# theislab/dca

Measured on AMD Instinct MI355X. Metric: cells/sec training (ZINB AE, 68k x 20k), higher is better.
Workload: dtype f32

## Files before the change

dca_amd/build.py:

```python
import os
import shutil
import subprocess
import sys

HERE = os.path.dirname(os.path.abspath(__file__))
ROOT = os.path.dirname(HERE)
CSRC = os.path.join(HERE, 'csrc')
LIB = os.path.join(CSRC, 'libdcahip.so')
SOURCES = ['dcahip_zinb.hip', 'dcahip_gemm.hip', 'dcahip_layers.hip', 'dcahip_heads.hip', 'dcahip_prep.hip', 'dcahip_opt.hip',
           'dcahip_dropout.hip', 'dcahip_sparse.hip', 'dcahip_peer.hip', 'dcahip_knn.hip', 'dcahip_kmeans.hip', 'dcahip_gram.hip',
           'dcahip_silhouette.hip']
HEADERS = ['zinb_math.hpp', 'h2_math.hpp', 'philox.hpp', 'knn_dist.hpp']
ARCH = 'gfx950'
HOST_LIB = os.path.join(CSRC, 'libdcahost.so')
HOST_SOURCES = ['dcahost_tsv.cpp', 'dcahost_read.cpp']


def _hipcc():
    for c in (shutil.which('hipcc'), '/opt/rocm/bin/hipcc'):
        if c and os.path.exists(c):
            return c
    raise RuntimeError('hipcc not found: cannot build libdcahip.so')


def _deps():
    return [os.path.join(CSRC, s) for s in SOURCES + HEADERS] + [os.path.join(ROOT, 'include', 'dcahip.h')]


def source_fingerprint():
    import hashlib
    h = hashlib.sha256()
    for d in _deps():
        h.update(os.path.basename(d).encode())
        if os.path.exists(d):
            with open(d, 'rb') as f:
                h.update(f.read())
    return h.hexdigest()


def needs_build():
    if not os.path.exists(LIB):
        return True
    t = os.path.getmtime(LIB)
    if any(os.path.exists(d) and os.path.getmtime(d) > t for d in _deps()):
        return True
    try:
        with open(LIB + '.src') as f:
            return f.read().strip() != source_fingerprint()
    except OSError:
        return True


def _obj_path(src, tag):
    return os.path.join(CSRC, '_obj', os.path.basename(src) + ('.' + tag if tag else '') + '.o')


def _obj_fingerprint(src, hdrs, defines):
    import hashlib
    h = hashlib.sha256()
    for d in [src] + list(hdrs):
        h.update(os.path.basename(d).encode())
        with open(d, 'rb') as f:
            h.update(f.read())
    h.update('\0'.join(defines).encode())
    return h.hexdigest()
# ... 74 lines not shown
```

dca_amd/config.py:

```python
import os
from dataclasses import dataclass, fields


def _flag(name, default):
    v = os.environ.get(name)
    return default if v is None else v not in ('0', '', 'off', 'false', 'False')


@dataclass
class EngineConfig:
    stack: str = 'steps'
    bwd_chain: bool = True
    wide_planes: bool = True
    wide_h2: bool = True
    dp_sharded_opt: bool = False
    dp_graph: bool = True
    dp_peer_exchange: bool = False
    device_prep: bool = True
    fused_write: bool = True
    resident: str = 'auto'
    counts_compact: bool = False
    graph_steps: int = 8
    sparse_dw_min: int = 512
    lut_fwd_min: int = 1024
    enc0_nt_min: int = 256
    predict_chunk: int = 1024

    _ENV = {'stack': 'DCA_AMD_STACK', 'bwd_chain': 'DCA_AMD_BWD_CHAIN', 'wide_planes': 'DCA_AMD_WIDE_PLANES', 'wide_h2': 'DCA_AMD_WIDE_H2',
            'dp_sharded_opt': 'DCA_AMD_DP_SHARDED_OPT', 'dp_graph': 'DCA_AMD_DP_GRAPH', 'device_prep': 'DCA_AMD_DEVICE_PREP',
            'fused_write': 'DCA_AMD_FUSED_WRITE', 'dp_peer_exchange': 'DCA_AMD_DP_PEER', 'resident': 'DCA_AMD_RESIDENT',
            'counts_compact': 'DCA_AMD_COUNTS_COMPACT'}

    @classmethod
    def from_env(cls):
        c = cls()
        for f in fields(cls):
            env = cls._ENV.get(f.name)
            if env is None:
                continue
            if f.type is bool or isinstance(getattr(c, f.name), bool):
                setattr(c, f.name, _flag(env, getattr(c, f.name)))
            elif os.environ.get(env) is not None:
                setattr(c, f.name, type(getattr(c, f.name))(os.environ[env]))
        if c.stack not in ('steps', 'coop', 'off'):
            raise ValueError('DCA_AMD_STACK must be steps, coop or off (got %r)' % c.stack)
        if c.resident not in ('auto', 'counts', 'dense'):
            raise ValueError('DCA_AMD_RESIDENT must be auto, counts or dense (got %r)' % c.resident)
        return c


def current():
    return EngineConfig.from_env()
```

dca_amd/csrc/dcahip_heads.hip:

```cpp
#include <hip/hip_runtime.h>
#include <stdint.h>
#include <type_traits>
#include "dcahip.h"
#include "zinb_math.hpp"

namespace {

using f32x16 = __attribute__((ext_vector_type(16))) float;

constexpr int kTG = 32;
constexpr int kTR = 32;
constexpr int kLdS = 33;
constexpr int kWG = 2;
constexpr int kMaxGrid = 2048;
constexpr int kMaxSmallGrid = 8192;
constexpr int kCUs = 256;
constexpr int kZU = 4;
constexpr int kQCap = 320;

__device__ __forceinline__ int rowmap(int e, int hi) { return (e & 3) + 8 * (e >> 2) + 4 * hi; }

__device__ __forceinline__ void wave_sync() {
    __builtin_amdgcn_fence(__ATOMIC_RELEASE, "wavefront");
    __builtin_amdgcn_wave_barrier();
    __builtin_amdgcn_fence(__ATOMIC_ACQUIRE, "wavefront");
}

using f16x8 = __attribute__((ext_vector_type(8))) _Float16;
using f16x2v = __attribute__((ext_vector_type(2))) _Float16;
using f32x2v = __attribute__((ext_vector_type(2))) float;
using u32x4 = __attribute__((ext_vector_type(4))) unsigned;
using u32x2 = __attribute__((ext_vector_type(2))) unsigned;
using s16x4 = __attribute__((ext_vector_type(4))) short;

constexpr int kWR2 = 8;
constexpr int kWr8MinNT = 5;
constexpr int kHTile = 2 * 32 * 64;
constexpr int kTop = 13;
constexpr int kDExp0 = 8;
constexpr float kDLim = 30000.f;
constexpr int kDSlack = 2;
constexpr int kEHZero = 64;

#define MFMAH(a, b, c) __builtin_amdgcn_mfma_f32_32x32x16_f16(__builtin_bit_cast(f16x8, a), __builtin_bit_cast(f16x8, b), c, 0, 0, 0)

__device__ __forceinline__ unsigned pk_f16(float a, float b) {
    return __builtin_bit_cast(unsigned, __builtin_convertvector(f32x2v{a, b}, f16x2v));
}
__device__ __forceinline__ float resid_lo(unsigned p, float x) {
    float r;
    asm("v_fma_mix_f32 %0, %1, -1.0, %2 op_sel:[0,0,0] op_sel_hi:[1,0,0]" : "=v"(r) : "v"(p), "v"(x));
    return r;
}
__device__ __forceinline__ float resid_hi(unsigned p, float x) {
    float r;
    asm("v_fma_mix_f32 %0, %1, -1.0, %2 op_sel:[1,0,0] op_sel_hi:[1,0,0]" : "=v"(r) : "v"(p), "v"(x));
    return r;
// ... 711 lines not shown
#pragma unroll
                for (int h = 0; h < NH; ++h) bsum[h] += rs[(n++) * 64];
                thsum += rs[(n++) * 64];
            }
            __syncthreads();
        }
    }
    if (r == 0 && tile_ok) {
        const bool direct = p.S == 1;
        float* out = direct ? p.gW : p.ws_dw + (long)s * p.dw_stride;
        const long ldo = direct ? p.ldg : p.ldws;
        const float fin = direct ? p.inv_n : 1.f;
        const bool cw = gene < p.plane;
#pragma unroll
        for (int h = 0; h < NH; ++h) {
#pragma unroll
            for (int ib = 0; ib < 2; ++ib)
#pragma unroll
                for (int e = 0; e < 16; ++e) {
                    const int i = ib * 32 + rowmap(e, hi);
                    if (cw && i < p.hL) out[(long)i * ldo + (long)h * p.plane + gene] = dW[h][ib][e] * fin;
                }
            const float bv = bsum[h] + __shfl_xor(bsum[h], 32, 64);
            if (cw && hi == 0) out[(long)p.hL * ldo + (long)h * p.plane + gene] = bv * fin;
        }
        if (CONST_DISP) {
            const float tv = thsum + __shfl_xor(thsum, 32, 64);
            if (direct) {
                if (gvalid && hi == 0) {
                    const float e = expf(p.theta_w[gene]);
                    p.g_theta[gene] = (e >= 1e-3f && e <= 1e4f) ? tv * p.inv_n * e : 0.f;
                }
            } else if (cw && hi == 0) {
                out[(long)(p.hL + 1) * ldo + gene] = tv;
            }
        }
    }
    __syncthreads();
    first_item = false;
    }

#pragma unroll
    for (int off = 32; off > 0; off >>= 1) dacc += __shfl_down(dacc, off, 64);
    if (lane == 0) lred[wave] = dacc;
    __syncthreads();
    if (tid == 0) {
        double v = 0.0;
        for (int w = 0; w < WR; ++w) v += lred[w];
        p.partials[blockIdx.x] = v;
    }
}


struct ReduceDwArgs {
    const float* ws; int S; long stride; int hL; long ldws, ncols; float* gW; long ldg;
    const float* theta_w; float* g_theta; int G;
    float scale;
    const float* ws2; int S2; const int* tail_tiles; int ntail; long plane;
    int tail_first;
};

__device__ __forceinline__ void reduce_dw_body(const ReduceDwArgs& q, int bid, int nblk) {
    const int hL = q.hL;
    const long ldws = q.ldws, ncols = q.ncols; float* gW = q.gW; const long ldg = q.ldg;
    const float* theta_w = q.theta_w; float* g_theta = q.g_theta; const int G = q.G;
    const float sc = q.scale;
    __shared__ unsigned tailbm[kMaxGrid / 32];
    if (q.ntail > 0) {
        for (int i = threadIdx.x; i < kMaxGrid / 32; i += 256) tailbm[i] = 0u;
        __syncthreads();
        for (int i = threadIdx.x; i < q.ntail; i += 256) {
            const int tl = q.tail_tiles ? q.tail_tiles[i] : q.tail_first + i;
            if (tl >= 0 && tl < kMaxGrid) atomicOr(&tailbm[tl >> 5], 1u << (tl & 31));
        }
        __syncthreads();
    }
    auto is_tail = [&](long col_in_plane) { const int tl = (int)(col_in_plane / kTG); return q.ntail > 0 && ((tailbm[tl >> 5] >> (tl & 31)) & 1u); };
    if ((ncols & 3) == 0 && (ldws & 3) == 0 && (ldg & 3) == 0 && (q.stride & 3) == 0 && (q.plane & 3) == 0 &&
        ((reinterpret_cast<uintptr_t>(q.ws) | reinterpret_cast<uintptr_t>(gW) | reinterpret_cast<uintptr_t>(q.ws2)) & 15) == 0) {
        const long nq = ncols >> 2, totalq = (long)(hL + 1) * nq;
        for (long idx = (long)bid * 256 + threadIdx.x; idx < totalq; idx += (long)nblk * 256) {
            const long i = idx / nq, c = (idx - i * nq) << 2;
            const bool tl = is_tail(c % q.plane);
            const float* ws = tl ? q.ws2 : q.ws; const int S = tl ? q.S2 : q.S; const long stride = q.stride;
            float4 v = *reinterpret_cast<const float4*>(ws + i * ldws + c);
            for (int s = 1; s < S; ++s) {
                const float4 x = *reinterpret_cast<const float4*>(ws + (long)s * stride + i * ldws + c);
                v.x += x.x; v.y += x.y; v.z += x.z; v.w += x.w;
            }
            v.x *= sc; v.y *= sc; v.z *= sc; v.w *= sc;
            *reinterpret_cast<float4*>(gW + i * ldg + c) = v;
        }
    } else {
        const long total = (long)(hL + 1) * ncols;
        for (long idx = (long)bid * 256 + threadIdx.x; idx < total; idx += (long)nblk * 256) {
            const long i = idx / ncols, c = idx - i * ncols;
            const bool tl = is_tail(c % q.plane);
            const float* ws = tl ? q.ws2 : q.ws; const int S = tl ? q.S2 : q.S;
            float v = 0.f;
            for (int s = 0; s < S; ++s) v += ws[(long)s * q.stride + i * ldws + c];
            gW[i * ldg + c] = v * sc;
        }
    }
    if (g_theta) {
        for (long c = (long)bid * 256 + threadIdx.x; c < G; c += (long)nblk * 256) {
            const bool tl = is_tail(c);
            const float* ws = tl ? q.ws2 : q.ws; const int S = tl ? q.S2 : q.S; const long stride = q.stride;
            float v = 0.f;
            for (int s = 0; s < S; ++s) v += ws[(long)s * stride + (long)(hL + 1) * ldws + c];
            const float e = expf(theta_w[c]);
            g_theta[c] = (e >= 1e-3f && e <= 1e4f) ? v * sc * e : 0.f;
        }
    }
}

__global__ __launch_bounds__(256) void heads_reduce_dw_kernel(ReduceDwArgs q) { reduce_dw_body(q, blockIdx.x, gridDim.x); }

struct ReduceDhArgs {
    const float* ws; int ntg, B, Bpad, KT, hL; float* dH; long lddh; float scale;
    const double* loss_partials; int n_partials; double loss_scale; float* loss_out;
    const float* ws2; int ntg2;
};

template <int GL>
__device__ __forceinline__ void reduce_dh_body(const ReduceDhArgs& q, int bid) {
    const float* ws = q.ws; const int ntg = q.ntg, B = q.B, KT = q.KT, hL = q.hL; float* dH = q.dH; const long lddh = q.lddh;
    const double* loss_partials = q.loss_partials; const int n_partials = q.n_partials; const double loss_scale = q.loss_scale;
    float* loss_out = q.loss_out;
    constexpr int OUT = 256 / GL;
    __shared__ float4 red[256];
    const int o = threadIdx.x % OUT, gl = threadIdx.x / OUT;
    const int q4 = KT / 4;
    const long nq = (long)B * q4;
    const long quad = (long)bid * OUT + o;
    float4 v = make_float4(0.f, 0.f, 0.f, 0.f);
    if (quad < nq) {
        const long tq = (long)kTR * q4;
        const long t = quad / tq, within = quad - t * tq;
        const float4* src = reinterpret_cast<const float4*>(ws) + t * ntg * tq + within;
        for (int gt0 = gl; gt0 < ntg; gt0 += 8 * GL) {
            float4 x[8];
#pragma unroll
            for (int u = 0; u < 8; ++u) {
                const int gt = gt0 + u * GL;
                x[u] = src[(long)(gt < ntg ? gt : gl) * tq];
            }
#pragma unroll
            for (int u = 0; u < 8; ++u)
                if (gt0 + u * GL < ntg) { v.x += x[u].x; v.y += x[u].y; v.z += x[u].z; v.w += x[u].w; }
        }
        if (q.ntg2 > 0) {
            const float4* src2 = reinterpret_cast<const float4*>(q.ws2) + t * q.ntg2 * tq + within;
            for (int gt = gl; gt < q.ntg2; gt += GL) { const float4 x = src2[(long)gt * tq]; v.x += x.x; v.y += x.y; v.z += x.z; v.w += x.w; }
        }
    }
    red[threadIdx.x] = v;
    __syncthreads();
    if (gl == 0 && quad < nq) {
#pragma unroll
        for (int k = 1; k < GL; ++k) {
            const float4 x = red[k * OUT + o];
            v.x += x.x; v.y += x.y; v.z += x.z; v.w += x.w;
        }
        const long row = quad / q4;
        const int i = (int)(quad - row * q4) * 4;
        float* d = dH + row * lddh + i;
        if (i + 0 < hL) d[0] = v.x * q.scale;
        if (i + 1 < hL) d[1] = v.y * q.scale;
        if (i + 2 < hL) d[2] = v.z * q.scale;
        if (i + 3 < hL) d[3] = v.w * q.scale;
    }
    if (loss_out && bid == 0) {
        __shared__ double lsum[256];
        double a = 0.0;
        for (int i = threadIdx.x; i < n_partials; i += 256) a += loss_partials[i];
        lsum[threadIdx.x] = a;
        __syncthreads();
        for (int st = 128; st > 0; st >>= 1) {
            if ((int)threadIdx.x < st) lsum[threadIdx.x] += lsum[threadIdx.x + st];
            __syncthreads();
        }
        if (threadIdx.x == 0) {
            float lf = (float)(lsum[0] * loss_scale);
            if (isnan(lf)) lf = INFINITY;
            *loss_out = lf;
        }
    }
}

template <int GL>
__global__ __launch_bounds__(256) void heads_reduce_dh_kernel(ReduceDhArgs q) { reduce_dh_body<GL>(q, blockIdx.x); }

template <int GL>
__global__ __launch_bounds__(256) void heads_reduce_both_kernel(ReduceDhArgs qh, ReduceDwArgs qw, int n_dh) {
    if ((int)blockIdx.x < n_dh) reduce_dh_body<GL>(qh, blockIdx.x);
    else reduce_dw_body(qw, blockIdx.x - n_dh, gridDim.x - n_dh);
}


struct HeadsPlan {
    bool small;
    int HLB, WR, S, NT, ntg, ngb, grid;
    int nitems, npart;
    long ldws, dw_stride, dw_bytes, dh_bytes, hs_bytes;
    int nmain, ntail, S2, grid2, npart2, nitems2;
    long dh2_bytes, dw2_bytes;
};

inline bool al16(const void* p) { return (reinterpret_cast<uintptr_t>(p) & 15) == 0; }

bool make_heads_plan(int B, int hL, int G, long plane, int flags, HeadsPlan* out) {
    if (flags & (DCAHIP_NLL_POISSON | DCAHIP_NLL_MSE)) return false;
    if (B <= 0 || G <= 0 || hL <= 0 || hL > 64 || plane < G || (plane & 3) || plane > ((G + 31) & ~31)) return false;
    if (B > (1 << 22)) return false;
    const bool has_pi = flags & DCAHIP_NLL_HAS_PI, cdisp = flags & DCAHIP_NLL_CONST_DISP;
    const int NH = 1 + (cdisp ? 0 : 1) + (has_pi ? 1 : 0);
    HeadsPlan p;
    p.HLB = 2;
    p.NT = (B + kTR - 1) / kTR;
    p.ntg = (G + kTG - 1) / kTG;
    p.ngb = p.ntg;
    if (p.ngb > kMaxGrid) return false;
    p.small = p.NT < kWr8MinNT;
    static_assert((kWr8MinNT - 1) * kMaxGrid <= kMaxSmallGrid, "loss partials of the four-wave kernel");
    p.WR = p.small ? 1 : kWR2;
    const int smax = (p.NT + p.WR - 1) / p.WR;
    double best = 1e300;
    p.S = 1;
    const double item_cost = 0.75;
    for (int S = 1; S <= smax && (long)S * p.ngb <= kMaxGrid; ++S) {
        const long items = (long)S * p.ngb;
        const long rounds = (items + kCUs - 1) / kCUs;
        const int tiles = (p.NT + S * p.WR - 1) / (S * p.WR);
        const double cost = (double)rounds * (tiles + item_cost);
        if (cost < best - 1e-9) { best = cost; p.S = S; }
    }
    p.nitems = p.S * p.ngb;
    p.grid = p.nitems;
    p.npart = p.ntg;
    if (p.small) {
        p.S = p.NT;
        p.nitems = p.NT * p.ntg;
        p.grid = p.nitems;
        p.npart = p.ntg;
    } else {
        const int res = kCUs / p.S * p.S;
        if (p.grid > res) p.grid = res;
        p.npart = p.grid / p.S;
    }
// ... 441 lines not shown
        }
    const int ea = block_exp(wave_max(ma)), eb = block_exp(wave_max(mb));
    const float sa = pow2i(ea), sb = pow2i(eb);
    f32x16 acc;
#pragma unroll
    for (int e = 0; e < 16; ++e) acc[e] = 0.f;
    for (int k0 = 0; k0 < K; k0 += 16) {
        float av[8], bv[8];
#pragma unroll
        for (int j = 0; j < 8; ++j) {
            av[j] = A[(long)l31 * K + k0 + 8 * hi + j] * sa;
            bv[j] = B[(long)(k0 + 8 * hi + j) * 32 + l31] * sb;
        }
        u32x4 af[2], bf[2];
        split8(av, af);
        split8(bv, bf);
        MFMA_H3(af, bf, acc)
    }
    const float un = pow2i(-(ea + eb));
#pragma unroll
    for (int e = 0; e < 16; ++e) C[rowmap(e, hi) * 32 + l31] = acc[e] * un;
}

template <bool P, bool C, bool YC>
void launch_fused(const HeadsPlan& pl, const HeadsArgs2& a, hipStream_t s) {
    if (pl.small) hipLaunchKernelGGL((heads_fused_small_kernel<P, C, YC>), dim3(pl.grid), dim3(256), 0, s, a);
    else hipLaunchKernelGGL((heads_fused_h2_kernel<P, C, YC>), dim3(pl.grid), dim3(64 * kWR2), 0, s, a);
}

}

extern "C" long dcahip_heads_fused_workspace_bytes(int B, int hL, int G, long plane, int flags) {
    HeadsPlan p;
    if (!make_heads_plan(B, hL, G, plane, flags, &p)) return 0;
    long need = 0;
    for (int nt = 1; nt <= p.NT; ++nt) {
        const int b = nt * kTR < B ? nt * kTR : B;
        HeadsPlan q;
        if (!make_heads_plan(b, hL, G, plane, flags, &q)) continue;
        const long n = q.dw_bytes + q.dh_bytes + q.hs_bytes + q.dw2_bytes + q.dh2_bytes;
        if (n > need) need = n;
    }
    return need;
}

extern "C" int dcahip_x3_product_32x32(const float* A, const float* B, float* C, int K, void* stream) {
    if (!A || !B || !C || K <= 0 || (K & 15)) return DCAHIP_EINVAL;
    hipLaunchKernelGGL(x3_product_kernel, dim3(1), dim3(64), 0, static_cast<hipStream_t>(stream), A, B, C, K);
    return (int)hipGetLastError();
}

extern "C" int dcahip_heads_tile_order_len(int G) { return G > 0 ? (((G + kTG - 1) / kTG + kWG - 1) / kWG) * kWG : 0; }

extern "C" int dcahip_heads_fused(const float* H, long ldh, const float* Wh, long ldw,
                                  const float* bh, long plane, const float* theta_w,
                                  const float* y, long ldy,
                                  const unsigned char* yc, long ldc, const int* ovf_ptr, const int* ovf_col,
                                  const float* ovf_val, const float* sf, const int* perm,
                                  const long long* cursor, int B, int hL, int G, float ridge,
                                  float inv_n, int flags, float* gW, long ldg, float* g_theta,
                                  float* dH, long lddh, double* loss_partials, int* n_partials_out,
                                  void* workspace, long workspace_bytes, const int* tile_order,
                                  float* loss_out, int d_exp, void* stream) {
    const bool has_pi = flags & DCAHIP_NLL_HAS_PI, cdisp = flags & DCAHIP_NLL_CONST_DISP;
    HeadsPlan pl;
    if (!make_heads_plan(B, hL, G, plane, flags, &pl)) return DCAHIP_EINVAL;
    if (!H || !Wh || !bh || (!y && !yc) || !sf || !gW || !dH || !loss_partials || !workspace) return DCAHIP_EINVAL;
    if (cdisp && (!theta_w || !g_theta)) return DCAHIP_EINVAL;
    if (workspace_bytes < pl.dw_bytes + pl.dh_bytes + pl.hs_bytes + pl.dw2_bytes + pl.dh2_bytes) return DCAHIP_EINVAL;
    if (!al16(H) || !al16(Wh) || !al16(workspace) || (ldh & 3) || (ldw & 3) || ldh < ((hL + 3) & ~3))
        return DCAHIP_EINVAL;
    if (d_exp > 0 || d_exp < -24 || !(ridge >= 0.f) || ridge > 1e3f) return DCAHIP_EINVAL;
    const int NH = 1 + (cdisp ? 0 : 1) + (has_pi ? 1 : 0);
    if (ldw < (long)NH * plane || ldg < (long)NH * plane) return DCAHIP_EINVAL;
    if (yc ? (ldc < G || ldc > 0xffffffffL) : (ldy < G || ldy > 0xffffffffL)) return DCAHIP_EINVAL;
    float* ws_dh = static_cast<float*>(workspace);
    float* ws_dw = ws_dh + pl.dh_bytes / sizeof(float);
    float* ws_dh2 = ws_dw + pl.dw_bytes / sizeof(float);
    float* ws_dw2 = ws_dh2 + pl.dh2_bytes / sizeof(float);
    hipStream_t s = static_cast<hipStream_t>(stream);
    bool direct_dw = false;
    {
        unsigned short* HA = reinterpret_cast<unsigned short*>(reinterpret_cast<char*>(workspace) + pl.dh_bytes + pl.dw_bytes +
                                                               pl.dh2_bytes + pl.dw2_bytes);
        unsigned short* HT = HA + (long)pl.NT * kHTile;
        int* eH = reinterpret_cast<int*>(HT + (long)pl.NT * kHTile);
        if (!pl.small) {
            hipLaunchKernelGGL(heads_split_h_kernel, dim3(pl.NT), dim3(256), 0, s, H, ldh, B, hL, HA, HT, eH);
            int rc0 = (int)hipGetLastError();
            if (rc0 != 0) return rc0;
        }
        direct_dw = pl.S == 1;
        HeadsArgs2 a{HA, HT, eH, H, ldh, gW, ldg, g_theta, Wh, ldw, bh, theta_w, y, ldy, yc, ldc, ovf_ptr, ovf_col, ovf_val,
                     sf, perm, cursor, ws_dw, pl.dw_stride, ws_dh,
                     pl.npart, pl.nitems, tile_order, loss_partials, plane, pl.ldws, B, hL, G, pl.S, pl.NT, ridge, inv_n, d_exp, 0};
        auto launch = [&](const HeadsPlan& q, const HeadsArgs2& b) {
            if (yc) {
                if (has_pi && cdisp) launch_fused<true, true, true>(q, b, s);
                else if (has_pi) launch_fused<true, false, true>(q, b, s);
                else if (cdisp) launch_fused<false, true, true>(q, b, s);
                else launch_fused<false, false, true>(q, b, s);
            } else {
                if (has_pi && cdisp) launch_fused<true, true, false>(q, b, s);
                else if (has_pi) launch_fused<true, false, false>(q, b, s);
                else if (cdisp) launch_fused<false, true, false>(q, b, s);
                else launch_fused<false, false, false>(q, b, s);
            }
        };
        launch(pl, a);
        if (pl.ntail > 0) {
            HeadsPlan q2 = pl;
            q2.grid = pl.grid2; q2.S = pl.S2;
            HeadsArgs2 b = a;
            b.ws_dw = ws_dw2; b.ws_dh = ws_dh2; b.npart = pl.npart2; b.nitems = pl.nitems2; b.S = pl.S2;
            b.partials = loss_partials + pl.grid; b.tile_base = pl.nmain;
            launch(q2, b);
        }
    }
    int rc = (int)hipGetLastError();
    if (rc != 0) return rc;
    const int n_part = pl.grid + pl.grid2;
    if (n_partials_out) *n_partials_out = n_part;
    {
        const int KT = pl.HLB * 32;
        const long nq = (long)B * (KT / 4);
        const ReduceDhArgs qh{ws_dh, pl.npart, B, pl.NT * kTR, KT, hL, dH, lddh, inv_n, loss_partials, n_part, (double)inv_n, loss_out,
                              ws_dh2, pl.npart2};
        const long total = (long)(hL + 1) * pl.ldws;
        long gr = (total / 4 + 255) / 256;
        if (gr > 2048) gr = 2048;
        if (gr < 1) gr = 1;
        const ReduceDwArgs qw{ws_dw, pl.S, pl.dw_stride, hL, pl.ldws, pl.ldws, gW, ldg, cdisp ? theta_w : nullptr,
                              cdisp ? g_theta : nullptr, G, inv_n,
                              ws_dw2, pl.S2, (pl.ntail > 0 && tile_order) ? tile_order + pl.nmain : nullptr, pl.ntail, plane, pl.nmain};
        const int gl = (nq <= 1024 && pl.npart >= 256) ? 64 : (nq >= 64L * 512 ? 4 : 16);
        const int n_dh = (int)((nq + 256 / gl - 1) / (256 / gl));
        if (!direct_dw) {
            const dim3 grid(n_dh + (int)gr);
            if (gl == 64) hipLaunchKernelGGL(heads_reduce_both_kernel<64>, grid, dim3(256), 0, s, qh, qw, n_dh);
            else if (gl == 4) hipLaunchKernelGGL(heads_reduce_both_kernel<4>, grid, dim3(256), 0, s, qh, qw, n_dh);
            else hipLaunchKernelGGL(heads_reduce_both_kernel<16>, grid, dim3(256), 0, s, qh, qw, n_dh);
        } else {
            if (gl == 64) hipLaunchKernelGGL(heads_reduce_dh_kernel<64>, dim3(n_dh), dim3(256), 0, s, qh);
            else if (gl == 4) hipLaunchKernelGGL(heads_reduce_dh_kernel<4>, dim3(n_dh), dim3(256), 0, s, qh);
            else hipLaunchKernelGGL(heads_reduce_dh_kernel<16>, dim3(n_dh), dim3(256), 0, s, qh);
        }
        rc = (int)hipGetLastError();
    }
    return rc;
}
```

dca_amd/csrc/dcahip_layers.hip:

```cpp
#include <hip/hip_runtime.h>
#include <stdint.h>
#include "dcahip.h"

namespace {

constexpr int kMaxChunks = 256;
constexpr int kApplyRows = 16;

constexpr float kSeluScale = 1.0507009873554805f, kSeluAlpha = 1.6732632423543772f;
constexpr int kActPre = 12;

__device__ __attribute__((noinline)) float act_fwd_other(int a, float x) {
    switch (a) {
        case 2: return tanhf(x);
        case 3: { const float e = expf(-fabsf(x)); const float s = 1.f / (1.f + e); return x >= 0.f ? s : e * s; }
        case 4: return x > 0.f ? x : expm1f(x);
        case 5: return kSeluScale * (x > 0.f ? x : kSeluAlpha * expm1f(x));
        case 6: return fmaxf(x, 0.f) + log1pf(expf(-fabsf(x)));
        case 7: return x / (1.f + fabsf(x));
        case 10: return fminf(fmaxf(0.2f * x + 0.5f, 0.f), 1.f);
        case 11: return expf(x);
        case 12: { const float e = expf(-fabsf(x)); const float s = 1.f / (1.f + e); return x * (x >= 0.f ? s : e * s); }
        case 13: return 0.5f * x * (1.f + erff(x * 0.70710678118654752f));
        default: return x > 0.f ? x : 0.3f * x;
    }
}
__device__ __forceinline__ float act_fwd(int a, float x) {
    if (a == 1) return fmaxf(x, 0.f);
    if (a == 0) return x;
    return act_fwd_other(a, x);
}

__device__ __attribute__((noinline)) float act_grad_other(int a, float v) {
    switch (a) {
        case 2: return 1.f - v * v;
        case 3: return v * (1.f - v);
        case 4: return v > 0.f ? 1.f : v + 1.f;
        case 5: return v > 0.f ? kSeluScale : v + kSeluScale * kSeluAlpha;
        case 6: return -expm1f(-v);
        case 7: { const float t = 1.f - fabsf(v); return t * t; }
        case 10: return v > 0.f && v < 1.f ? 0.2f : 0.f;
        case 11: return v;
        case 12: {
            const float e = expf(-fabsf(v)); const float s0 = 1.f / (1.f + e); const float s = v >= 0.f ? s0 : e * s0;
            return s * (1.f + v * (1.f - s));
        }
        case 13:
            return 0.5f * (1.f + erff(v * 0.70710678118654752f)) + v * 0.39894228040143268f * expf(-0.5f * v * v);
        default: return v > 0.f ? 1.f : 0.3f;
    }
}
__device__ __forceinline__ float act_grad(int a, float h) {
    if (a == 1) return h > 0.f ? 1.f : 0.f;
    if (a == 0) return 1.f;
    return act_grad_other(a, h);
// ... 795 lines not shown
                    const int r = wg + kBwdWGs * (ty + 4 * j);
                    acc[j] = fmaf(r < a.B ? dZs[r][c] : 0.f, w, acc[j]);
                }
            }
#pragma unroll
            for (int j = 0; j < NR; ++j) {
                const int r = wg + kBwdWGs * (ty + 4 * j);
                if (r < a.B) a.dHp[(long)r * a.lddp + k] = acc[j];
            }
        }
    }
}

__global__ __launch_bounds__(256) void relu_bwd_kernel(const float* dH, long ldd, const float* Hact,
                                                       long ldh, int B, int H, float* dZ, long ldz, int act) {
    const long total = (long)B * H;
    for (long i = (long)blockIdx.x * 256 + threadIdx.x; i < total; i += (long)gridDim.x * 256) {
        const int r = (int)(i / H), c = (int)(i - (long)r * H);
        dZ[(long)r * ldz + c] = dH[(long)r * ldd + c] * act_grad(act, Hact[(long)r * ldh + c]);
    }
}

__global__ __launch_bounds__(256) void relu_fwd_kernel(const float* Z, long ldz, int B, int H,
                                                       float* Hout, long ldh, int act) {
    const long total = (long)B * H;
    for (long i = (long)blockIdx.x * 256 + threadIdx.x; i < total; i += (long)gridDim.x * 256) {
        const int r = (int)(i / H), c = (int)(i - (long)r * H);
        Hout[(long)r * ldh + c] = act_fwd(act, Z[(long)r * ldz + c]);
    }
}

__global__ __launch_bounds__(256) void colsum_chain_kernel(const float* x, long ldx, int B, int N,
                                                           const float* theta_w, float* out) {
    __shared__ float sm[256];
    const int tx = threadIdx.x & 63, ty = threadIdx.x >> 6;
    const int c = blockIdx.x * 64 + tx;
    float s = 0.f;
    if (c < N) for (int i = ty; i < B; i += 4) s += x[(long)i * ldx + c];
    const float tot = wg_rowlane_sum(s, sm);
    if (c < N && ty == 0) {
        float chain = 1.f;
        if (theta_w) {
            const float e = expf(theta_w[c]);
            chain = (e >= 1e-3f && e <= 1e4f) ? e : 0.f;
        }
        out[c] = tot * chain;
    }
}

struct StepEnd {
    const float* loss; double weight; float* hist; int rows_per_slot; double* acc; long long* cursor; int advance; int on;
};

__global__ __launch_bounds__(256) void rmsprop_clip_kernel(float* w, const float* g, float* ms,
                                                           long n, const float* lrp, float rho,
                                                           float eps, float clip, StepEnd se) {
    if (se.on && blockIdx.x == 0 && threadIdx.x == 0) {
        const long long c = se.cursor ? *se.cursor : 0;
        if (se.loss) {
            const float l = *se.loss;
            if (se.hist) se.hist[se.rows_per_slot > 0 ? c / se.rows_per_slot : 0] = l;
            if (se.acc) *se.acc += (double)l * se.weight;
        }
        if (se.cursor) *se.cursor = c + se.advance;
    }
    const float lr = *lrp;
    const long nv = n >> 2;
    const long stride = (long)gridDim.x * 256;
    for (long i = (long)blockIdx.x * 256 + threadIdx.x; i < nv; i += stride) {
        float4 gv = reinterpret_cast<const float4*>(g)[i];
        float4 mv = reinterpret_cast<const float4*>(ms)[i];
        float4 wv = reinterpret_cast<const float4*>(w)[i];
        float* gp = &gv.x; float* mp = &mv.x; float* wp = &wv.x;
#pragma unroll
        for (int j = 0; j < 4; ++j) {
            float gj = gp[j];
            if (clip > 0.f) gj = fminf(fmaxf(gj, -clip), clip);
            mp[j] = rho * mp[j] + (1.f - rho) * gj * gj;
            wp[j] = wp[j] - lr * gj / (sqrtf(mp[j]) + eps);
        }
        reinterpret_cast<float4*>(ms)[i] = mv;
        reinterpret_cast<float4*>(w)[i] = wv;
    }
    for (long i = (nv << 2) + (long)blockIdx.x * 256 + threadIdx.x; i < n; i += stride) {
        float gj = g[i];
        if (clip > 0.f) gj = fminf(fmaxf(gj, -clip), clip);
        const float m = rho * ms[i] + (1.f - rho) * gj * gj;
        ms[i] = m;
        w[i] = w[i] - lr * gj / (sqrtf(m) + eps);
    }
}

__global__ __launch_bounds__(256) void transpose_kernel(const float* __restrict__ src, long lds_, int R, int C,
                                                        float* __restrict__ dst, long ldd,
                                                        const int* __restrict__ perm, const long long* __restrict__ cursor) {
    __shared__ float tile[32][33];
    const int tx = threadIdx.x & 31, ty = threadIdx.x >> 5;
    const int r0 = blockIdx.y * 32, c0 = blockIdx.x * 32;
    const long long cur = (perm && cursor) ? *cursor : 0;
#pragma unroll
    for (int k = 0; k < 4; ++k) {
        const int r = r0 + ty + 8 * k, c = c0 + tx;
        float v = 0.f;
        if (r < R && c < C) {
            const long sr = perm ? (long)perm[cur + r] : (long)r;
            v = src[sr * lds_ + c];
        }
        tile[ty + 8 * k][tx] = v;
    }
    __syncthreads();
#pragma unroll
    for (int k = 0; k < 4; ++k) {
        const int c = c0 + ty + 8 * k, r = r0 + tx;
        if (c < C && r < R) dst[(long)c * ldd + r] = tile[tx][ty + 8 * k];
    }
}

__global__ __launch_bounds__(256) void transpose64_kernel(const float* __restrict__ src, long lds_, int R, int C,
                                                          float* __restrict__ dst, long ldd,
                                                          const int* __restrict__ perm, const long long* __restrict__ cursor) {
    __shared__ float tile[64][65];
    const int tq = threadIdx.x & 15, tr = threadIdx.x >> 4;
    const int r0 = blockIdx.y * 64, c0 = blockIdx.x * 64;
    const long long cur = (perm && cursor) ? *cursor : 0;
    float4 v[4];
#pragma unroll
    for (int k = 0; k < 4; ++k) {
        const int r = r0 + tr + 16 * k, c = c0 + 4 * tq;
        const int rc = r < R ? r : R - 1;
        const long sr = perm ? (long)perm[cur + rc] : (long)rc;
        v[k] = *reinterpret_cast<const float4*>(src + sr * lds_ + (c < C ? c : 0));
    }
#pragma unroll
    for (int k = 0; k < 4; ++k) {
        const int r = tr + 16 * k, c = 4 * tq;
        tile[r][c] = v[k].x; tile[r][c + 1] = v[k].y; tile[r][c + 2] = v[k].z; tile[r][c + 3] = v[k].w;
    }
    __syncthreads();
#pragma unroll
    for (int k = 0; k < 4; ++k) {
        const int c = tr + 16 * k, r = 4 * tq;
        if (c0 + c < C) {
// ... 176 lines not shown
                if (L.xhat) L.xhat[(long)(r0 + r) * L.ldx + c] = xh;
                L.Hout[(long)(r0 + r) * L.ldh + c] = h;
                ht[r * kStackLd + c] = h;
            }
        }
        if (i + 1 == a.n) break;
        const SmallLayer& N = a.l[i + 1];
        const int K = H, HN = N.H;
        for (int idx = tid; idx < ((K + 3) & ~3) * 64; idx += 256) {
            const int k = idx >> 6, cc = idx & 63;
            wl[k * kStackLd + cc] = (k < K && cc < HN) ? N.W[(long)k * N.ldw + cc] : 0.f;
        }
        for (int idx = tid; idx < kStackRows * 4; idx += 256) {
            const int r = idx >> 2, kk = (K & ~3) + (idx & 3);
            if (kk >= K && kk < ((K + 3) & ~3)) ht[r * kStackLd + kk] = 0.f;
        }
        __syncthreads();
        float acc[kStackRows / 4];
#pragma unroll
        for (int j = 0; j < kStackRows / 4; ++j) acc[j] = 0.f;
        const int K4 = (K + 3) & ~3;
        for (int k = 0; k < K4; k += 4) {
            const float w0 = wl[(k + 0) * kStackLd + c], w1 = wl[(k + 1) * kStackLd + c];
            const float w2 = wl[(k + 2) * kStackLd + c], w3 = wl[(k + 3) * kStackLd + c];
#pragma unroll
            for (int j = 0; j < kStackRows / 4; ++j) {
                const int r = ty + 4 * j;
                if (r < nrows) {
                    const float4 h4 = *reinterpret_cast<const float4*>(ht + r * kStackLd + k);
                    acc[j] = fmaf(h4.w, w3, fmaf(h4.z, w2, fmaf(h4.y, w1, fmaf(h4.x, w0, acc[j]))));
                }
            }
        }
        __syncthreads();
        if (c < HN) {
            const float b = N.bias ? N.bias[c] : 0.f;
#pragma unroll
            for (int j = 0; j < kStackRows / 4; ++j) {
                const int r = ty + 4 * j;
                if (r < nrows) {
                    const float z = acc[j] + b;
                    zt[r * kStackLd + c] = z;
                    if (N.Z) N.Z[(long)(r0 + r) * N.ldz + c] = z;
                }
            }
        }
        __syncthreads();
        block_stats(i + 1);
        fresh = true;
    }
    if (nbar) grid_exit(a.sync, (unsigned)nwg);
}

__global__ __launch_bounds__(256) void hidden_stack_bwd_kernel(StackBwdArgs a) {
    __shared__ __attribute__((aligned(16))) float dyt[kStackRows * kStackLd];
    __shared__ __attribute__((aligned(16))) float xt[kStackRows * kStackLd];
    __shared__ __attribute__((aligned(16))) float ht[kStackRows * kStackLd];
    __shared__ __attribute__((aligned(16))) float wl[64 * kStackLd];
    __shared__ float smf[256];
    const int tid = threadIdx.x, tx = tid & 63, ty = tid >> 6;
    const int wg = blockIdx.x, nwg = a.nwg;
    const int cr = chunk_rows(a.B, nwg);
    const int r0 = wg * cr;
    const int nrows = max(0, min(a.B, r0 + cr) - r0);
    const int c = tx;
    unsigned nbar = 0;
    auto prep = [&](int i, bool load_dh, bool with_sums) {
        const StackBwdLayer& L = a.l[i];
        const int H = L.H;
        if (load_dh) {
            for (int r = ty; r < kStackRows; r += 4)
                dyt[r * kStackLd + tx] = (r < nrows && tx < H) ? L.dHin[(long)(r0 + r) * L.lddh + tx] : 0.f;
        }
        float s1 = 0.f, s2 = 0.f;
        const float bc = c < H ? pre_beta(a.act, L.beta, c) : 0.f;
        if (c < H)
            for (int r = ty; r < nrows; r += 4) {
                const float h = L.Hact[(long)(r0 + r) * L.ldh + c];
                const float xh = L.xhat[(long)(r0 + r) * L.ldx + c];
                const float dy = dyt[r * kStackLd + c] * act_slope(a.act, h, xh, bc);
                dyt[r * kStackLd + c] = dy;
                xt[r * kStackLd + c] = xh;
                s1 += dy; s2 += dy * xh;
            }
        if (!with_sums) { __syncthreads(); return; }
        const float t1 = wg_rowlane_sum(s1, smf);
        const float t2 = wg_rowlane_sum(s2, smf);
        float* part = a.part + (long)i * nwg * 2 * 64;
        if (c < H && ty == 0) {
            part[((long)wg * 2 + 0) * H + c] = t1;
            part[((long)wg * 2 + 1) * H + c] = t2;
        }
    };
    bool fresh = false, have_tile = false;
    if (a.first == 0) { prep(a.n - 1, true, true); fresh = true; have_tile = true; }
    for (int step = max(a.first, 1); step <= min(a.last, a.n); ++step) {
        const int i = a.n - step;
        const StackBwdLayer& L = a.l[i];
        const int H = L.H;
        if (!have_tile) { prep(i, true, false); have_tile = true; }
        if (fresh) grid_barrier(a.sync, (unsigned)nwg * (++nbar));
        const float* part = a.part + (long)i * nwg * 2 * 64;
        float v1 = 0.f, v2 = 0.f;
        {
            const int cc = c < H ? c : H - 1;
            for (int e0 = ty; e0 < nwg; e0 += 64) {
// ... 34 lines not shown
        {
            float acc[16];
#pragma unroll
            for (int j = 0; j < 16; ++j) acc[j] = 0.f;
            float bs = 0.f;
            for (int r = 0; r < nrows; ++r) {
                const float d = dyt[r * kStackLd + c];
                bs += d;
#pragma unroll
                for (int q4 = 0; q4 < 4; ++q4) {
                    const float4 h4 = *reinterpret_cast<const float4*>(ht + r * kStackLd + 16 * ty + 4 * q4);
                    acc[4 * q4 + 0] = fmaf(h4.x, d, acc[4 * q4 + 0]); acc[4 * q4 + 1] = fmaf(h4.y, d, acc[4 * q4 + 1]);
                    acc[4 * q4 + 2] = fmaf(h4.z, d, acc[4 * q4 + 2]); acc[4 * q4 + 3] = fmaf(h4.w, d, acc[4 * q4 + 3]);
                }
            }
#pragma unroll
            for (int j = 0; j < 16; ++j) {
                const int k = 16 * ty + j;
                if (k < K) gw[(long)k * 64 + c] = acc[j];
            }
            if (ty == 0) gw[(long)K * 64 + c] = bs;
        }
        {
            float acc[kStackRows / 4];
#pragma unroll
            for (int j = 0; j < kStackRows / 4; ++j) acc[j] = 0.f;
            for (int c4 = 0; c4 < 64; c4 += 4) {
                const float4 w4 = *reinterpret_cast<const float4*>(wl + tx * kStackLd + c4);
#pragma unroll
                for (int j = 0; j < kStackRows / 4; ++j) {
                    const int r = ty + 4 * j;
                    if (r < nrows) {
                        const float4 d4 = *reinterpret_cast<const float4*>(dyt + r * kStackLd + c4);
                        acc[j] = fmaf(d4.w, w4.w, fmaf(d4.z, w4.z, fmaf(d4.y, w4.y, fmaf(d4.x, w4.x, acc[j]))));
                    }
                }
            }
            __syncthreads();
            const StackBwdLayer& P = a.l[i - 1];
#pragma unroll
            for (int j = 0; j < kStackRows / 4; ++j) {
                const int r = ty + 4 * j;
                const float v = (r < nrows && tx < K) ? acc[j] : 0.f;
                dyt[r * kStackLd + tx] = v;
                if (r < nrows && tx < K && P.dHin) P.dHin[(long)(r0 + r) * P.lddh + tx] = v;
            }
        }
        __syncthreads();
        prep(i - 1, false, true);
        fresh = true;
    }
    if (a.last > a.n) {
        if (fresh) grid_barrier(a.sync, (unsigned)nwg * (++nbar));
        for (int i = 1; i < a.n; ++i) {
            const StackBwdLayer& L = a.l[i];
            const int total = (L.K + 1) * L.H;
            const float* gw = a.gwp + (long)i * nwg * 65 * 64;
            const int el = tid & 31, sl = tid >> 5;
            const int per = (nwg + 7) / 8;
            for (int e0 = wg * 32; e0 < total; e0 += nwg * 32) {
                const int e = e0 + el;
                const int ec = e < total ? e : total - 1;
                const int k = ec / L.H, cc = ec - k * L.H;
                const float* src = gw + (long)k * 64 + cc;
                float v = 0.f;
                for (int b0 = sl * per; b0 < min(nwg, (sl + 1) * per); b0 += 16) {
                    float pv[16];
#pragma unroll
                    for (int u = 0; u < 16; ++u) pv[u] = src[(long)min(b0 + u, nwg - 1) * 65 * 64];
#pragma unroll
                    for (int u = 0; u < 16; ++u) if (b0 + u < min(nwg, (sl + 1) * per)) v += pv[u];
                }
                __syncthreads();
                smf[tid] = v;
                __syncthreads();
                if (tid < 32 && e < total) {
                    float t = 0.f;
#pragma unroll
                    for (int q8 = 0; q8 < 8; ++q8) t += smf[q8 * 32 + tid];
                    L.gW[(long)k * L.ldg + cc] = t;
                }
            }
        }
    }
    if (nbar) grid_exit(a.sync, (unsigned)nwg);
}

__device__ __forceinline__ bool w_tile_vec(const float* W, long ldw, int H) {
    return (H & 3) == 0 && (ldw & 3) == 0 && (reinterpret_cast<uintptr_t>(W) & 15) == 0;
}
template <int VEC = 0>
__device__ __forceinline__ void w_tile_request(const float* W, long ldw, int K, int H, int tid, float4 (&wv)[4]) {
    if (VEC == 0 && (!W || K <= 0)) {
#pragma unroll
        for (int q = 0; q < 4; ++q) wv[q] = make_float4(0.f, 0.f, 0.f, 0.f);
        return;
    }
    const bool vec = VEC == 1 || (VEC == 0 && w_tile_vec(W, ldw, H));
    if (vec) {
#pragma unroll
        for (int q = 0; q < 4; ++q) {
            const int idx = tid + 256 * q, k = min(idx >> 4, K - 1), c4 = min((idx & 15) * 4, H - 4);
            wv[q] = *reinterpret_cast<const float4*>(W + (long)k * ldw + c4);
        }
    } else {
#pragma unroll
        for (int q = 0; q < 4; ++q) {
            const int idx = tid + 256 * q, k = min(idx >> 4, K - 1), c4 = (idx & 15) * 4;
            const float* src = W + (long)k * ldw;
            wv[q].x = src[min(c4 + 0, H - 1)]; wv[q].y = src[min(c4 + 1, H - 1)];
            wv[q].z = src[min(c4 + 2, H - 1)]; wv[q].w = src[min(c4 + 3, H - 1)];
        }
    }
}
__device__ __forceinline__ void w_tile_store(float* wl, int K, int H, int tid, const float4 (&wv)[4]) {
#pragma unroll
    for (int q = 0; q < 4; ++q) {
        const int idx = tid + 256 * q, k = idx >> 4, c4 = (idx & 15) * 4;
        float4 v = wv[q];
        if (k >= K || c4 + 0 >= H) v.x = 0.f;
        if (k >= K || c4 + 1 >= H) v.y = 0.f;
        if (k >= K || c4 + 2 >= H) v.z = 0.f;
        if (k >= K || c4 + 3 >= H) v.w = 0.f;
        *reinterpret_cast<float4*>(wl + k * kStackLd + c4) = v;
    }
}

constexpr int kStepRows = 32;

struct StepFwdArgs {
    SmallLayer cur, nxt;
    int B, act, nwg, stats_only;
    float momentum, eps;
    const float* part_in;
    float* part_out;
    const float* ext_in; const float* ext_counts; int ext_E;
};

// ... 75 lines not shown
            float h = 0.f;
            if (r < nrows && c < H) {
                const float xh = bn_xhat(z[j], mean, inv);
                h = act_fwd(a.act, xh + beta);
                if (L.xhat) L.xhat[(long)(r0 + r) * L.ldx + c] = xh;
                L.Hout[(long)(r0 + r) * L.ldh + c] = h;
            }
            ht[r * kStackLd + c] = h;
        }
        if (!N.W) return;
        w_tile_store(wl, K, HN, tid, wv);
        __syncthreads();
        float acc[kStepRows / 4];
#pragma unroll
        for (int j = 0; j < kStepRows / 4; ++j) acc[j] = 0.f;
        tile_fwd<kStepRows / 4, kStackLd, kStackLd, 0>(acc, wl, ht, (K + 3) & ~3, tx, ty);
        Hs = HN;
#pragma unroll
        for (int j = 0; j < kStepRows / 4; ++j) {
            const int r = ty + 4 * j;
            out_z[j] = acc[j] + nbias;
            if (r < nrows && c < HN && N.Z) N.Z[(long)(r0 + r) * N.ldz + c] = out_z[j];
        }
    } else {
#pragma unroll
        for (int j = 0; j < kStepRows / 4; ++j) out_z[j] = z[j];
    }
    float sv = 0.f;
#pragma unroll
    for (int j = 0; j < kStepRows / 4; ++j) if (ty + 4 * j < nrows && c < Hs) sv += out_z[j];
    const float tot = wg_rowlane_sum(sv, smf);
    const float bmean = nrows > 0 ? tot / (float)nrows : 0.f;
    float q = 0.f;
#pragma unroll
    for (int j = 0; j < kStepRows / 4; ++j) if (ty + 4 * j < nrows && c < Hs) { const float d = out_z[j] - bmean; q += d * d; }
    const float bm2 = wg_rowlane_sum(q, smf);
    if (c < Hs && ty == 0) {
        a.part_out[((long)wg * 2 + 0) * Hs + c] = bmean;
        a.part_out[((long)wg * 2 + 1) * Hs + c] = bm2;
    }
}

struct StepBwdArgs {
    StackBwdLayer cur, low;
    int B, act, nwg, sums_only;
    float n_total;
    float* dZ0; long ldz0;
    const float* part_in;
    float* part_out;
    float* gwp;
    const float* ext_in;
};

__global__ __launch_bounds__(256) void stack_bwd_step_kernel(StepBwdArgs a) {
    __shared__ __attribute__((aligned(16))) float dyt[kStepRows * kStackLd];
    __shared__ __attribute__((aligned(16))) float ht[kStepRows * kStackLd];
    __shared__ __attribute__((aligned(16))) float wl[64 * kStackLd];
    __shared__ float smf[256];
    const int tid = threadIdx.x, tx = tid & 63, ty = tid >> 6;
    const int wg = blockIdx.x, E = a.nwg;
    const int cr = chunk_rows(a.B, E);
    const int r0 = wg * cr;
    const int nrows = max(0, min(a.B, r0 + cr) - r0);
    const int c = tx;
    const StackBwdLayer& L = a.cur;
    const int H = L.H, cc = c < H ? c : H - 1;
    float dh[kStepRows / 4], hv[kStepRows / 4], xv[kStepRows / 4];
#pragma unroll
    for (int j = 0; j < kStepRows / 4; ++j) {
        const int r = ty + 4 * j;
        const long row = r0 + (r < nrows ? r : (nrows > 0 ? nrows - 1 : 0));
        dh[j] = L.dHin[row * L.lddh + cc]; hv[j] = L.Hact[row * L.ldh + cc]; xv[j] = L.xhat[row * L.ldx + cc];
    }
    float dy[kStepRows / 4];
    const float bc = pre_beta(a.act, L.beta, cc);
    if (a.sums_only) {
        float s1 = 0.f, s2 = 0.f;
        tile_dy_sums(dy, xv, c < H, nrows, ty, [&](int j) { return dh[j] * act_slope(a.act, hv[j], xv[j], bc); }, s1, s2);
        const float t1 = wg_rowlane_sum(s1, smf), t2 = wg_rowlane_sum(s2, smf);
        if (c < H && ty == 0) { a.part_out[((long)wg * 2 + 0) * H + c] = t1; a.part_out[((long)wg * 2 + 1) * H + c] = t2; }
        return;
    }
    const float* const ein = a.ext_in ? a.ext_in : a.part_in;
    const int Em = a.ext_in ? 1 : E;
    float p1[16], p2[16];
#pragma unroll
    for (int u = 0; u < 16; ++u) {
        const long eo = (long)(ty + 4 * u < Em ? ty + 4 * u : Em - 1) * 2;
        p1[u] = ein[(eo + 0) * H + cc]; p2[u] = ein[(eo + 1) * H + cc];
    }
    const bool has_low = a.low.Hact != nullptr;
    const int K = has_low ? L.K : 0;
    float4 wv[4];
    float hp[kStepRows / 4];
    w_tile_request(has_low ? L.W : nullptr, L.ldw, K, H, tid, wv);
#pragma unroll
    for (int j = 0; j < kStepRows / 4; ++j) {
        const int r = ty + 4 * j;
        const long row = r0 + (r < nrows ? r : (nrows > 0 ? nrows - 1 : 0));
        const int kc = tx < K ? tx : (K > 0 ? K - 1 : 0);
        hp[j] = has_low ? L.Hprev[row * L.ldp + kc] : 0.f;
    }
    const float inv = L.inv_std[cc];
    float v1 = 0.f, v2 = 0.f;
#pragma unroll
    for (int u = 0; u < 16; ++u) if (ty + 4 * u < Em && c < H) { v1 += p1[u]; v2 += p2[u]; }
#pragma unroll 1
    for (int e0 = ty + 64; e0 < Em; e0 += 64) {
        float q1[16], q2[16];
#pragma unroll
        for (int u = 0; u < 16; ++u) {
            const long eo = (long)(e0 + 4 * u < Em ? e0 + 4 * u : Em - 1) * 2;
            q1[u] = ein[(eo + 0) * H + cc]; q2[u] = ein[(eo + 1) * H + cc];
// ... 10 lines not shown
        const int r = ty + 4 * j;
        float dz = 0.f;
        if (r < nrows && c < H) {
            dz = bn_dz(inv, dh[j] * act_slope(a.act, hv[j], xv[j], bc), xv[j], m1, m2);
            if (!has_low) a.dZ0[(long)(r0 + r) * a.ldz0 + c] = dz;
        }
        dyt[r * kStackLd + c] = dz;
        ht[r * kStackLd + tx] = (r < nrows && tx < K) ? hp[j] : 0.f;
    }
    if (!has_low) return;
    w_tile_store(wl, K, H, tid, wv);
    __syncthreads();
    float lh[kStepRows / 4], lx[kStepRows / 4];
#pragma unroll
    for (int j = 0; j < kStepRows / 4; ++j) {
        const int r = ty + 4 * j;
        const long row = r0 + (r < nrows ? r : (nrows > 0 ? nrows - 1 : 0));
        const int kc = tx < K ? tx : (K > 0 ? K - 1 : 0);
        lh[j] = a.low.Hact[row * a.low.ldh + kc];
        lx[j] = a.low.xhat[row * a.low.ldx + kc];
    }
    float* gw = a.gwp + (long)wg * 65 * 64;
    {
        float acc[16];
#pragma unroll
        for (int j = 0; j < 16; ++j) acc[j] = 0.f;
        float bs = 0.f;
        tile_dw<kStackLd, 2>(acc, bs, dyt, ht, nrows, tx, ty);
#pragma unroll
        for (int j = 0; j < 16; ++j) {
            const int k = 16 * ty + j;
            if (k < K) gw[(long)k * 64 + c] = acc[j];
        }
        if (ty == 0) gw[(long)K * 64 + c] = bs;
    }
    float acc[kStepRows / 4];
#pragma unroll
    for (int j = 0; j < kStepRows / 4; ++j) acc[j] = 0.f;
    tile_dhp<kStepRows / 4, kStackLd, 2>(acc, wl, dyt, tx, ty);
    const StackBwdLayer& P = a.low;
    const float pbc = pre_beta(a.act, P.beta, tx < K ? tx : (K > 0 ? K - 1 : 0));
    float s1 = 0.f, s2 = 0.f;
#pragma unroll
    for (int j = 0; j < kStepRows / 4; ++j) {
        const int r = ty + 4 * j;
        if (r < nrows && tx < K) {
            P.dHin[(long)(r0 + r) * P.lddh + tx] = acc[j];
            const float d = acc[j] * act_slope(a.act, lh[j], lx[j], pbc);
            s1 += d; s2 += d * lx[j];
        }
    }
    const float t1 = wg_rowlane_sum(s1, smf), t2 = wg_rowlane_sum(s2, smf);
    if (tx < K && ty == 0) { a.part_out[((long)wg * 2 + 0) * K + tx] = t1; a.part_out[((long)wg * 2 + 1) * K + tx] = t2; }
}

struct ChainBwdArgs {
    StackBwdLayer l[4];
    int B, act;
    float n_total;
    float* dZ0; long ldz0;
};

template <int NL, int R, bool VEC>
__global__ __launch_bounds__(256) void stack_bwd_chain_kernel(ChainBwdArgs a) {
    __shared__ __attribute__((aligned(16))) float dyt[4 * R * kStackLd];
    __shared__ __attribute__((aligned(16))) float ht[4 * R * kStackLd];
    __shared__ __attribute__((aligned(16))) float wl[64 * kStackLd];
    __shared__ float smf[256];
    const int tid = threadIdx.x, tx = tid & 63, ty = tid >> 6;
    const int nrows = a.B, c = tx;
    float hv[NL][R], xv[NL][R], inv[NL], dh[R];
    float4 wv[NL][4];
    {
        const StackBwdLayer& T = a.l[NL - 1];
        const int cc = c < T.H ? c : T.H - 1;
#pragma unroll
        for (int j = 0; j < R; ++j) {
            const int r = ty + 4 * j;
            dh[j] = T.dHin[(long)(r < nrows ? r : nrows - 1) * T.lddh + cc];
        }
    }
#pragma unroll
    for (int t = 0; t < NL; ++t) {
        const int i = NL - 1 - t;
        const StackBwdLayer& L = a.l[i];
        const int cc = c < L.H ? c : L.H - 1;
#pragma unroll
        for (int j = 0; j < R; ++j) {
            const int r = ty + 4 * j;
            const long row = r < nrows ? r : nrows - 1;
            hv[i][j] = L.Hact[row * L.ldh + cc]; xv[i][j] = L.xhat[row * L.ldx + cc];
        }
        inv[i] = L.inv_std[cc];
        if (i > 0) w_tile_request<VEC ? 1 : 2>(L.W, L.ldw, L.K, L.H, tid, wv[i]);
    }
#pragma unroll
    for (int t = 0; t < NL; ++t) {
        const int i = NL - 1 - t;
        const StackBwdLayer& L = a.l[i];
        const int H = L.H, K = i > 0 ? L.K : 0;
        float dy[R], s1 = 0.f, s2 = 0.f;
        if (a.act == 1) {
#pragma unroll
            for (int j = 0; j < R; ++j) dy[j] = hv[i][j] > 0.f ? dh[j] : 0.f;
        } else {
            const float bc = pre_beta(a.act, L.beta, c < H ? c : H - 1);
// ... 375 lines not shown
    if (!a_mean || !k || !c || !a_pi || B <= 0 || G <= 0 || lda < G || ldp < G) return DCAHIP_EINVAL;
    const int gy = B < 64 ? B : 64;
    hipLaunchKernelGGL(elempi_fwd_kernel, dim3((G + 255) / 256, gy), dim3(256), 0, static_cast<hipStream_t>(stream),
                       a_mean, lda, k, c, B, G, a_pi, ldp);
    return (int)hipGetLastError();
}

extern "C" int dcahip_elempi_bwd(const float* m, long lda, float* d_mean, const float* d_pi, long ldd, const float* k,
                                 int B, int G, float* gk, float* gc, double* workspace, void* stream) {
    if (!m || !d_mean || !d_pi || !k || !gk || !gc || !workspace || B <= 0 || G <= 0 || lda < G || ldd < G)
        return DCAHIP_EINVAL;
    const int R = B < kElemPiSlices ? B : kElemPiSlices;
    hipStream_t s = static_cast<hipStream_t>(stream);
    hipLaunchKernelGGL(elempi_bwd_kernel, dim3((G + 255) / 256, R), dim3(256), 0, s, m, lda, d_mean, d_pi, ldd, k, B, G,
                       workspace);
    hipLaunchKernelGGL(elempi_finish_kernel, dim3((G + 255) / 256), dim3(256), 0, s, workspace, R, G, gk, gc);
    return (int)hipGetLastError();
}

extern "C" int dcahip_bcast_cols(const float* s, long lds, int B, int G, float* out, long ldo, void* stream) {
    if (!s || !out || B <= 0 || G <= 0 || ldo < G || lds < 1) return DCAHIP_EINVAL;
    int gx = (G + 255) / 256;
    if (gx > 64) gx = 64;
    hipLaunchKernelGGL(bcast_cols_kernel, dim3(gx, B), dim3(256), 0, static_cast<hipStream_t>(stream), s, lds, B, G, out, ldo);
    return (int)hipGetLastError();
}

extern "C" int dcahip_row_sums_strided(const float* x, long ldx, int B, int G, float* out, long ldo, void* stream) {
    if (!x || !out || B <= 0 || G <= 0 || ldx < G || ldo < 1) return DCAHIP_EINVAL;
    hipLaunchKernelGGL(row_sums_strided_kernel, dim3((B + 3) / 4), dim3(256), 0, static_cast<hipStream_t>(stream),
                       x, ldx, B, G, out, ldo);
    return (int)hipGetLastError();
}

extern "C" int dcahip_colsum_chain(const float* x, long ldx, int B, int N, const float* theta_w,
                                   float* out, void* stream) {
    if (!x || !out || B <= 0 || N <= 0) return DCAHIP_EINVAL;
    hipLaunchKernelGGL(colsum_chain_kernel, dim3((N + 63) / 64), dim3(256), 0,
                       static_cast<hipStream_t>(stream), x, ldx, B, N, theta_w, out);
    return (int)hipGetLastError();
}

extern "C" int dcahip_rmsprop_clip(float* w, const float* g, float* ms, long n, const float* lr,
                                   float rho, float eps, float clip, const float* loss, double weight,
                                   float* hist, int rows_per_slot, double* acc, long long* cursor, int advance,
                                   void* stream) {
    if (!w || !g || !ms || !lr || n <= 0) return DCAHIP_EINVAL;
    if (!al16(w) || !al16(g) || !al16(ms)) return DCAHIP_EINVAL;
    long grid = ((n >> 2) + 255) / 256;
    if (grid > 2048) grid = 2048;
    if (grid < 1) grid = 1;
    hipLaunchKernelGGL(rmsprop_clip_kernel, dim3((int)grid), dim3(256), 0,
                       static_cast<hipStream_t>(stream), w, g, ms, n, lr, rho, eps, clip,
                       StepEnd{loss, weight, hist, rows_per_slot, acc, cursor, advance, (loss || hist || acc || cursor) ? 1 : 0});
    return (int)hipGetLastError();
}

extern "C" int dcahip_hidden_stack_max_rows(void) { return kStackMaxWG * kStackRows; }

extern "C" long dcahip_hidden_stack_workspace_bytes(int n_layers, int B) {
    if (n_layers < 1 || n_layers > kStackMaxLayers || B <= 0 || B > kStackMaxWG * kStackRows) return 0;
    const long nwg = stack_workgroups(B, 16);
    return 256 + ((long)n_layers * nwg * 2 * 64 + (long)n_layers * nwg * 65 * 64) * (long)sizeof(float);
}

static int stack_plan(int n, int B, int rows_per_wg, int first, int last, int nsteps, int* nwg_out) {
    if (rows_per_wg < 16 || rows_per_wg > kStackRows || first < 0 || last < first || last >= nsteps) return DCAHIP_EINVAL;
    const int nwg = stack_workgroups(B, rows_per_wg);
    if (nwg > kStackMaxPhaseWG) return DCAHIP_EINVAL;
    if (last > first && nwg > kStackMaxWG) return DCAHIP_EINVAL;
    *nwg_out = nwg;
    return 0;
}

static bool stack_shape_ok(const void* layers, int n, int B) {
    return layers && n >= 1 && n <= kStackMaxLayers && B > 0 && B <= kStackMaxWG * kStackRows;
}

static bool stack_workspace_ok(const void* workspace, long workspace_bytes, int n, int B) {
    return workspace && workspace_bytes >= dcahip_hidden_stack_workspace_bytes(n, B) && al16(workspace);
}

static bool stack_fwd_layers(const dcahip_small_layer* layers, int n, bool need_z, SmallLayer* l) {
    for (int i = 0; i < n; ++i) {
        const dcahip_small_layer& q = layers[i];
        if (q.H <= 0 || q.H > 64 || !q.Hout || !q.moving_mean || !q.moving_var) return false;
        if (i == 0 ? !q.Z : (!q.W || q.K != layers[i - 1].H || (need_z && !q.Z))) return false;
        l[i] = small_layer(q);
    }
    return true;
}

static bool stack_bwd_layers(const dcahip_stack_bwd_layer* layers, int n, int act, bool need_dh, StackBwdLayer* l) {
    for (int i = 0; i < n; ++i) {
        const dcahip_stack_bwd_layer& q = layers[i];
        if (q.H <= 0 || q.H > 64 || !q.Hact || !q.xhat || !q.inv_std || (act >= kActPre && !q.beta)) return false;
        if (i > 0 && (!q.W || !q.Hprev || !q.gW || q.K != layers[i - 1].H || q.K > 64)) return false;
        if (!q.dH && (i == n - 1 || need_dh)) return false;
        l[i] = StackBwdLayer{q.W, q.ldw, q.K, q.H, q.Hact, q.ldh, q.xhat, q.ldx, q.inv_std, q.Hprev, q.ldp, q.gW, q.ldg,
                             q.dbeta, q.dH, q.lddh, q.beta};
    }
    return true;
}

static StepFwdArgs stack_fwd_step(const SmallLayer* l, int n, int B, float momentum, float eps, int act, int step, int nwg,
                                  float* part) {
// ... 72 lines not shown
                                            void* workspace, long workspace_bytes, void* stream) {
    if (!stack_shape_ok(layers, n, B) || !dZ0 || !stack_workspace_ok(workspace, workspace_bytes, n, B)) return DCAHIP_EINVAL;
    if (step < 0 || step > n || (step > 0 && !ext_sums)) return DCAHIP_EINVAL;
    const int nwg = stack_workgroups(B, kStepRows);
    if (nwg > kStackMaxPhaseWG) return DCAHIP_EINVAL;
    StackBwdLayer l[kStackMaxLayers];
    if (!stack_bwd_layers(layers, n, act, true, l)) return DCAHIP_EINVAL;
    float* part = reinterpret_cast<float*>(static_cast<char*>(workspace) + 256);
    StepBwdArgs q = stack_bwd_step(l, n, B, n_total, act, dZ0, ldz0, step, nwg, part);
    if (step > 0) q.ext_in = ext_sums;
    hipStream_t st = static_cast<hipStream_t>(stream);
    hipLaunchKernelGGL(stack_bwd_step_kernel, dim3(nwg), dim3(256), 0, st, q);
    const int made = stack_bwd_made(n, step);
    if (made >= 0 && sums_out)
        hipLaunchKernelGGL(stack_sums_combine_kernel, dim3(1), dim3(64), 0, st, (const float*)q.part_out, nwg, l[made].H, sums_out,
                           l[made].dbeta);
    return (int)hipGetLastError();
}

extern "C" int dcahip_hidden_stack_bwd(const dcahip_stack_bwd_layer* layers, int n, int B, float n_total, int act,
                                       float* dZ0, long ldz0, int rows_per_wg, int first_step, int last_step,
                                       void* workspace, long workspace_bytes, void* stream) {
    if (!stack_shape_ok(layers, n, B) || !dZ0) return DCAHIP_EINVAL;
    const bool one_launch = first_step == 0 && last_step == n + 1;
    const bool chain = one_launch && B <= kStackRows && n <= 4;
    if (!chain && !stack_workspace_ok(workspace, workspace_bytes, n, B)) return DCAHIP_EINVAL;
    StackBwdArgs a{};
    if (stack_plan(n, B, rows_per_wg, first_step, last_step, n + 2, &a.nwg)) return DCAHIP_EINVAL;
    if (!stack_bwd_layers(layers, n, act, !one_launch, a.l)) return DCAHIP_EINVAL;
    a.n = n; a.B = B; a.act = act; a.first = first_step; a.last = last_step; a.n_total = n_total;
    a.dZ0 = dZ0; a.ldz0 = ldz0;
    if (chain) {
        ChainBwdArgs q{};
        for (int i = 0; i < n; ++i) q.l[i] = a.l[i];
        q.B = B; q.act = act; q.n_total = n_total; q.dZ0 = dZ0; q.ldz0 = ldz0;
        bool vec = true;
        for (int i = 1; i < n; ++i) vec = vec && (q.l[i].H & 3) == 0 && (q.l[i].ldw & 3) == 0 && al16(q.l[i].W);
        hipStream_t st = static_cast<hipStream_t>(stream);
        if (B <= 32) { if (vec) launch_bwd_chain<8, true>(n, q, st); else launch_bwd_chain<8, false>(n, q, st); }
        else { if (vec) launch_bwd_chain<16, true>(n, q, st); else launch_bwd_chain<16, false>(n, q, st); }
        return (int)hipGetLastError();
    }
    a.sync = static_cast<unsigned*>(workspace);
    a.part = reinterpret_cast<float*>(static_cast<char*>(workspace) + 256);
    a.gwp = a.part + (long)n * a.nwg * 2 * 64;
    if (first_step == last_step && first_step <= n && rows_per_wg == kStepRows) {
        const StepBwdArgs q = stack_bwd_step(a.l, n, B, n_total, act, dZ0, ldz0, first_step, a.nwg, a.part);
        hipLaunchKernelGGL(stack_bwd_step_kernel, dim3(a.nwg), dim3(256), 0, static_cast<hipStream_t>(stream), q);
        return (int)hipGetLastError();
    }
    hipLaunchKernelGGL(hidden_stack_bwd_kernel, dim3(a.nwg), dim3(256), 0, static_cast<hipStream_t>(stream), a);
    return (int)hipGetLastError();
}
```

dca_amd/engine.py:

```python
import math

import numpy as np
import torch

from . import prep as _prep

BN_MOMENTUM = 0.99
BN_EPS = 1e-3
RMS_RHO = 0.9
RMS_EPS = 1e-7

AE_HEADS = {
    'zinb-conddisp': (('mean', 'disp', 'pi'), False),
    'zinb': (('mean', 'pi'), True),
    'nb-conddisp': (('mean', 'disp'), False),
    'nb': (('mean',), True),
    'poisson': (('mean',), False),
    'normal': (('mean',), False),
    'nb-shared': (('mean', 'disp'), False, ('disp',)),
    'zinb-shared': (('mean', 'disp', 'pi'), False, ('disp', 'pi')),
    'nb-fork': (('mean', 'disp'), False, ()),
    'zinb-fork': (('mean', 'disp', 'pi'), False, ()),
}
AE_FORK = ('nb-fork', 'zinb-fork')
# ... 90 lines not shown
    def all_reduce_sum_async(self, t):
        return None

    def wait(self, work):
        pass


def _truncated_normal(rng, stddev, shape):
    out = rng.normal(0.0, 1.0, size=shape)
    bad = np.abs(out) > 2.0
    while bad.any():
        out[bad] = rng.normal(0.0, 1.0, size=int(bad.sum()))
        bad = np.abs(out) > 2.0
    return out * stddev


KERAS_INITIALIZERS = ('glorot_uniform', 'glorot_normal', 'he_uniform', 'he_normal', 'lecun_uniform', 'lecun_normal',
                      'random_uniform', 'random_normal', 'truncated_normal', 'orthogonal', 'zeros', 'ones')


def keras_initializer(name, rng, fan_in, fan_out, shape=None):
    key = name.lower() if isinstance(name, str) else name
    vs = {'glorot_uniform': (1.0, 'avg', 'u'), 'glorot_normal': (1.0, 'avg', 'n'),
          'he_uniform': (2.0, 'in', 'u'), 'he_normal': (2.0, 'in', 'n'),
          'lecun_uniform': (1.0, 'in', 'u'), 'lecun_normal': (1.0, 'in', 'n')}
    shape = (fan_in, fan_out) if shape is None else shape
    if key in vs:
        scale, mode, distr = vs[key]
        n = (fan_in + fan_out) / 2.0 if mode == 'avg' else float(fan_in)
        if distr == 'u':
            lim = math.sqrt(3.0 * scale / n)
            w = rng.uniform(-lim, lim, size=shape)
        else:
            w = _truncated_normal(rng, math.sqrt(scale / n) / .87962566103423978, shape)
    elif key == 'random_uniform':
        w = rng.uniform(-0.05, 0.05, size=shape)
    elif key == 'random_normal':
        w = rng.normal(0.0, 0.05, size=shape)
    elif key == 'truncated_normal':
        w = _truncated_normal(rng, 0.05, shape)
    elif key == 'orthogonal' and len(shape) == 2:
        a = rng.normal(0.0, 1.0, size=(max(shape), min(shape)))
        q, r = np.linalg.qr(a)
        q = q * np.sign(np.diag(r))
        w = q if fan_in >= fan_out else q.T
    elif key == 'zeros':
        w = np.zeros(shape)
    elif key == 'ones':
        w = np.ones(shape)
    else:
        raise NotImplementedError('init=%r is not implemented on the MI355X path (available: %s)'
                                  % (name, ', '.join(KERAS_INITIALIZERS)))
    return np.ascontiguousarray(w, dtype=np.float32)


class ParamLayout:

    def __init__(self, ae_type, input_size, output_size, hidden_size, batchnorm, prelu=False):
        self.ae_type = ae_type
        self.prelu = bool(prelu)
        self.heads, self.const_disp = AE_HEADS[ae_type][:2]
        self.shared = AE_HEADS[ae_type][2] if len(AE_HEADS[ae_type]) > 2 else ()
        self.elempi = ae_type in AE_ELEMPI
        self.dense_heads = tuple(h for h in self.heads if not (self.elempi and h == 'pi'))
        self.planes = tuple(h for h in self.dense_heads if h not in self.shared)
        self.G_in, self.G_out = input_size, output_size
        self.Gp = _r4(output_size)
        self.NH = len(self.planes) * self.Gp + (4 if self.shared else 0)
        self.ldA = self.NH + (len(self.shared) + (1 if self.elempi else 0)) * self.Gp
        self.hidden = tuple(int(h) for h in hidden_size)
        self.center = int(np.floor(len(self.hidden) / 2.0))
        self.fork = len(self.heads) if ae_type in AE_FORK else 0
        self.hfork = 0
        if self.fork:
            if len(self.hidden) - 1 <= self.center:
                raise ValueError('%s needs at least one hidden layer behind the centre (the reference fails with '
                                 'AttributeError: last_hidden_mean)' % ae_type)
            self.hfork = self.hidden[-1]
            self.hidden = self.hidden[:self.center + 1] + (self.fork * self.hfork,)
        self.batchnorm = batchnorm
        self.seg = {}
        off = 0

        def add(name, shape, align=False):
            nonlocal off
            if align:
                off = _r4(off)
            self.seg[name] = (off, shape)
            off += int(np.prod(shape))

        fan_in = input_size
        for i, h in enumerate(self.hidden):
            add('W%d' % i, (fan_in, h), align=True)
            add('b%d' % i, (h,))
            if batchnorm:
                add('beta%d' % i, (h,))
            if self.prelu:
                add('alpha%d' % i, (h,))
            fan_in = h
        self.hL = self.hfork if self.fork else fan_in
        add('Wh', (self.hL, self.NH), align=True)
        add('bh', (self.NH,))
        if self.const_disp:
            add('theta_w', (self.Gp,), align=True)
        if self.elempi:
            add('pi_k', (self.Gp,), align=True)
# ... 65 lines not shown
        self.mv = [torch.ones(h, **f32) for h in lay.hidden] if batchnorm else []
        self.lr = torch.full((1,), 1e-3, **f32)
        self.cursor = torch.zeros(1, dtype=torch.int64, device=self.dev)
        self.acc = torch.zeros(2, dtype=torch.float64, device=self.dev)
        self.partials = torch.zeros(ops.max_partials, dtype=torch.float64, device=self.dev)
        self.val_loss_tmp = torch.zeros(1, **f32)
        self.clip = 5.0
        self.ldD = lay.ldA + (lay.Gp if lay.const_disp else 0)
        self.Bmax = 0
        self._hl = None
        self.X = self.Y = self.sf = self.perm = None
        self.has_targets = False
        self.csr = None
        self.out_cols = self.col_out = None
        self.perm_id = self.cursor0 = None
        self.tile_order = None
        self.hist = None
        self.prof = None
        self.use_fused = not (lay.shared or lay.fork or lay.elempi)
        self.sharedpi = bool(sharedpi) and lay.elempi
        self.ws_elempi = torch.zeros(ops.elempi_workspace_doubles(lay.G_out), dtype=torch.float64, device=self.dev) \
            if lay.elempi else None
        self.ws_heads = None
        self._pending = None
        self.W0T = None
        self.WhT = self.HT = self.XT = self.dZT = None
        self.pl = None
        self.opt_kind = 'rmsprop'
        self.slot2 = None
        self.m_sched = None
        self.opt_iter = torch.zeros(1, dtype=torch.int64, device=self.dev)
        self.reg = None
        self.reg_ws = None
        self._counts_world_key = None
        self._counts_local, self._counts_world = {}, {}
        n_conf = len(tuple(hidden_size))
        hd = list(hidden_dropout) if isinstance(hidden_dropout, (list, tuple)) else [hidden_dropout] * n_conf
        assert len(hd) == n_conf
        if lay.fork:
            hd = hd[:lay.center + 1] + [hd[-1]]
        self.drop = [float(r) for r in hd]
        self.in_drop = float(input_dropout)
        assert all(0.0 <= r < 1.0 for r in self.drop + [self.in_drop]), 'dropout rates must be in [0, 1)'
        self.has_dropout = any(r > 0.0 for r in self.drop) or self.in_drop > 0.0
        self.drop_seed = int(dropout_seed) & (2 ** 64 - 1)
        self.drop_iter = torch.zeros(1, dtype=torch.int64, device=self.dev)
        self.row0 = 0
        self.Xb = None
        self.cc = self.cc_in = None
        self.cc_csr = None
        self._tile_lut = False
        self.ws_enc0 = self.ws_enc0l = None
        self.ws_stack = None
        self.stack_mode = self.cfg.stack
        self.sparse_dw_min = self.cfg.sparse_dw_min

    def _t(self, name):
        return self.prof.section(name) if self.prof is not None else _NULL

    @property
    def _kperm(self):
        return self.perm_id if self.csr is not None else self.perm

    @property
    def _kcur(self):
        return self.cursor0 if self.csr is not None else self.cursor

    @property
    def _dhl(self):
        return self.dH[-1] if self.lay.hidden else self.dHin0

    def init_params(self, seed=0, init='glorot_uniform'):
        rng = np.random.RandomState(seed)
        lay = self.lay
        p = {}
        fan_in = lay.G_in
        for i, h in enumerate(lay.hidden):
            if lay.fork and i == len(lay.hidden) - 1:
                p['W%d' % i] = np.concatenate([keras_initializer(init, rng, fan_in, lay.hfork)
                                               for _ in range(lay.fork)], axis=1)
            else:
                p['W%d' % i] = keras_initializer(init, rng, fan_in, h)
            fan_in = h
        for hd in lay.dense_heads:
            p['W_' + hd] = keras_initializer(init, rng, lay.hL, 1 if hd in lay.shared else lay.G_out)
        if lay.elempi:
            units = 1 if self.sharedpi else lay.G_out
            k = keras_initializer(init, rng, units, units, shape=(units,))
            p['pi_k'] = np.full(lay.G_out, k[0], np.float32) if self.sharedpi else k
        self.set_params(p)

    def set_params(self, p):
        lay = self.lay
        w = self.w.cpu()
        for name, (off, shape) in lay.seg.items():
            if name in ('Wh', 'bh', 'theta_w', 'pi_k', 'pi_c'):
                continue
            if name in p:
                w[off:off + int(np.prod(shape))] = torch.as_tensor(
                    np.asarray(p[name], dtype=np.float32).reshape(-1))
        Wh = lay.view(w, 'Wh'); bh = lay.view(w, 'bh')
        for hd in lay.dense_heads:
            c0, c1 = lay.head_cols(hd)
            if 'W_' + hd in p:
                Wh[:, c0:c1] = torch.as_tensor(np.asarray(p['W_' + hd], dtype=np.float32))
            if 'b_' + hd in p:
# ... 887 lines not shown
            self.counts_world = cw
            self._counts_world_key = key
        self.row0 = int(sum(world_counts[:self.comm.rank]))

    def assert_finite(self, where=''):
        lay = self.lay
        bad = []
        if not bool(torch.isfinite(self.g[lay.P]).item()):
            bad.append('loss')
        if not bool(torch.isfinite(self.g[:lay.P]).all().item()) or not bool(torch.isfinite(self.w[:lay.P]).all().item()):
            for name in lay.seg:
                for flat, kind in ((self.g, 'gradient of '), (self.w, '')):
                    if not bool(torch.isfinite(lay.view(flat, name)).all().item()):
                        bad.append(kind + name)
        if bad:
            raise FloatingPointError('dca: %s has inf/nans%s' % (', '.join(bad), (' (' + where + ')') if where else ''))

    def train_step(self, B, B_global=None, world_counts=None, rows_per_slot=None):
        lay, ops, comm = self.lay, self.ops, self.comm
        Bg = B if B_global is None else B_global
        inv_n = 1.0 / (float(Bg) * lay.G_out)
        w, g = self.w, self.g
        if comm.dp:
            self.set_world_counts(world_counts)
        if B > 0:
            if self.csr is not None:
                with self._t('csr_gather'):
                    self._gather_step(B)
            self._forward_backward(B, Bg, inv_n)
        else:
            self._empty_step()
        if comm.dp and self._use_sharded_opt():
            sh = self.flat_len // comm.world
            lo = comm.rank * sh
            comm.all_reduce_sum(g[lay.P:lay.P + 1])
            gs = comm.reduce_scatter_sum(g, self._g_shard(sh))
            n_upd = max(0, min(sh, lay.P - lo))
            if n_upd > 0:
                with self._t('rmsprop_clip'):
                    ops.rmsprop_clip(w[lo:lo + sh], gs, self.ms[lo:lo + sh], n_upd, self.lr, RMS_RHO, RMS_EPS, self.clip)
            comm.all_gather_into(w, w[lo:lo + sh])
            if self.has_dropout:
                ops.counter_add(self.drop_iter, 1)
            ops.step_end(g[lay.P:], float(Bg), self.hist, rows_per_slot or max(self.Bmax, 1), self.acc, self.cursor, B)
            return
        if comm.dp:
            comm.all_reduce_sum(g[:lay.seg['Wh'][0]])
            if self._pending is not None:
                comm.wait(self._pending)
                self._pending = None
        if self.reg is not None:
            ops.l1l2_apply(self.reg, w, g, g[lay.P:], self.reg_ws)
        fused_end = self.opt_kind == 'rmsprop' and not self.has_dropout and hasattr(ops, 'rmsprop_clip_end')
        if fused_end:
            with self._t('rmsprop_clip'):
                ops.rmsprop_clip_end(w, g, self.ms, lay.P, self.lr, RMS_RHO, RMS_EPS, self.clip, g[lay.P:], float(Bg),
                                     self.hist, rows_per_slot or max(self.Bmax, 1), self.acc, self.cursor, B)
            return
        if self.opt_kind == 'rmsprop':
            with self._t('rmsprop_clip'):
                ops.rmsprop_clip(w, g, self.ms, lay.P, self.lr, RMS_RHO, RMS_EPS, self.clip)
        elif self.opt_kind == 'nadam':
            ops.nadam_step(w, g, self.ms, self.slot2, lay.P, self.lr, self.opt_iter, self.m_sched, self.clip)
            ops.counter_add(self.opt_iter, 1)
        else:
            ops.optimizer_step(self.opt_kind, w, g, None if self.opt_kind == 'sgd' else self.ms,
                               self.slot2, lay.P, self.lr, self.opt_iter, self.clip)
            ops.counter_add(self.opt_iter, 1)
        if self.has_dropout:
            ops.counter_add(self.drop_iter, 1)
        ops.step_end(g[lay.P:], float(Bg), self.hist, rows_per_slot or max(self.Bmax, 1), self.acc,
                     self.cursor, B)

    def _heads_compact(self):
        kw = {'compact': self.cc} if self.cc is not None else {}
        if getattr(self, 'heads_d_exp', 0):
            kw['d_exp'] = self.heads_d_exp
        return kw

    def _use_sharded_opt(self):
        return self.sharded_opt and self.opt_kind == 'rmsprop' and self.reg is None

    def _g_shard(self, sh):
        if getattr(self, '_gshard', None) is None or self._gshard.numel() != sh:
            self._gshard = torch.zeros(sh, dtype=torch.float32, device=self.dev)
        return self._gshard

    def _launch_heads_bucket(self):
        if self.comm.dp and not self._use_sharded_opt():
            lay = self.lay
            self._pending = self.comm.all_reduce_sum_async(self.g[lay.seg['Wh'][0]:lay.P + 1])

    def _empty_step(self):
        lay = self.lay
        self.g.zero_()
        for i, h in enumerate(lay.hidden):
            if lay.batchnorm:
                entries, cnts, E = self._batch_moments(i, 0, h, self.counts_world)
                self.ops.bn_relu_apply(self.Z[i], self.ldh[i], 0, h, entries, cnts, E,
                                       lay.view(self.w, 'beta%d' % i), self.mm[i], self.mv[i],
                                       BN_MOMENTUM, BN_EPS, self.act, self.H[i], self.ldh[i], None, 0, None)
        self._launch_heads_bucket()
        for i in reversed(range(len(lay.hidden))):
            if lay.batchnorm:
                s = torch.zeros(2 * lay.hidden[i], dtype=torch.float32, device=self.dev)
                self.comm.all_reduce_sum(s)

    def heads_fused_launch(self, B, KL, inv_n):
        lay, w, g = self.lay, self.w, self.g
        self.ops.heads_fused(self._hl[0], self._hl[1], lay.view(w, 'Wh'), lay.NH,
                             lay.view(w, 'bh'), lay.Gp,
                             lay.view(w, 'theta_w') if lay.const_disp else None, self.Y,
                             self.ldy, self.sf, self._kperm, self._kcur, B, KL, lay.G_out,
                             self.ridge, inv_n, self.flags, lay.view(g, 'Wh'), lay.NH,
                             lay.view(g, 'theta_w') if lay.const_disp else None,
                             self._dhl, self._hl[1], self.partials, self.ws_heads,
                             tile_order=self.tile_order, loss_out=g[lay.P:], **self._heads_compact())

    def _forward_backward(self, B, Bg, inv_n):
        lay, ops, comm = self.lay, self.ops, self.comm
        w, g = self.w, self.g
        KL = self._hidden_forward(B, ('perm',), True, self.counts_world)
        self._last_heads_args = (B, KL, inv_n)
        if self.ws_heads is not None:
            with self._t('heads_fused'):
                self.heads_fused_launch(B, KL, inv_n)
        else:
            self._heads_backward_unfused(B, KL, inv_n)
        self._launch_heads_bucket()
        L = len(lay.hidden)
        chain = self._stack_chain(B)
        sync = self._stack_sync(B)
        coop = chain or sync or self._stack_coop(B)
        if coop:
            layers = []
            for i, h in enumerate(lay.hidden):
                d = dict(H=h, Hact=self.H[i], ldh=self.ldh[i], xhat=self.XH[i], ldx=self.ldh[i], inv_std=self.inv_std[i],
                         dbeta=lay.view(g, 'beta%d' % i), dH=self.dH[i], lddh=self.ldh[i], **self._pre_kw(i))
                if i > 0:
                    d.update(W=lay.view(w, 'W%d' % i), ldw=h, K=lay.hidden[i - 1], Hprev=self.H[i - 1], ldp=self.ldh[i - 1],
                             gW=lay.view(g, 'W%d' % i), ldg=h)
                layers.append(d)
            if sync:
                ops.hidden_stack_bwd_sync(layers, B, float(Bg), self.act, self.dZ[0], self.ldh[0], 0, None, self.bsum[L - 1],
                                          self.ws_stack)
                comm.all_reduce_sum(self.bsum[L - 1])
                for st in range(1, L + 1):
                    i = L - st
                    ops.hidden_stack_bwd_sync(layers, B, float(Bg), self.act, self.dZ[0], self.ldh[0], st, self.bsum[i],
                                              self.bsum[i - 1] if i > 0 else None, self.ws_stack)
                    if i > 0:
                        comm.all_reduce_sum(self.bsum[i - 1])
                ops.hidden_stack_bwd(layers, B, float(Bg), self.act, self.dZ[0], self.ldh[0], self.ws_stack,
                                     rows_per_wg=32, steps=(L + 1, L + 1))
            elif chain:
                ops.hidden_stack_bwd(layers, B, float(Bg), self.act, self.dZ[0], self.ldh[0], None, rows_per_wg=64)
            elif self.stack_mode == 'coop' and B <= 256 * 64:
                ops.hidden_stack_bwd(layers, B, float(Bg), self.act, self.dZ[0], self.ldh[0], self.ws_stack, rows_per_wg=64)
            else:
                for st in range(L + 2):
                    ops.hidden_stack_bwd(layers, B, float(Bg), self.act, self.dZ[0], self.ldh[0], self.ws_stack,
                                         rows_per_wg=self._stack_rows(B), steps=(st, st))
        for i in reversed(range(L)):
            if coop and i > 0:
                continue
            h = lay.hidden[i]
            if not coop:
                if self.drop[i] > 0.0:
                    ops.dropout_apply(self.dH[i], self.ldh[i], None, None, B, h, self.drop[i], self.drop_seed,
                                      self.drop_iter, i, self.row0, self.dH[i], self.ldh[i])
                if self.prelu:
                    ops.prelu_bwd(self.dH[i], self.ldh[i], self.H[i], self.ldh[i], lay.view(w, 'alpha%d' % i), B, h,
                                  lay.view(g, 'alpha%d' % i), self.ws_prelu)
                if self._layer_small(B, i):
                    Kp = lay.hidden[i - 1]
                    ops.dense_bn_bwd_small(self.dH[i], self.ldh[i], self._slope_in(i), self.ldh[i],
                                           self.XH[i] if lay.batchnorm else None, self.ldh[i], self.inv_std[i],
                                           self.Hcur[i - 1], self.ldh[i - 1], lay.view(w, 'W%d' % i), h, B, Kp, h,
                                           lay.batchnorm, float(Bg), self.act, lay.view(g, 'W%d' % i), h,
                                           lay.view(g, 'beta%d' % i) if lay.batchnorm else None,
                                           self.dH[i - 1], self.ldh[i - 1], **self._pre_kw(i))
                    continue
                if lay.batchnorm and self._bn_small(B):
                    ops.bn_bwd_small(self.dH[i], self.ldh[i], self.H[i], self.ldh[i], self.XH[i], self.ldh[i],
                                     self.inv_std[i], float(Bg), B, h, self.dZ[i], self.ldh[i],
                                     lay.view(g, 'beta%d' % i), self.act, **self._pre_kw(i))
                elif lay.batchnorm:
                    ops.bn_bwd_sums(self.dH[i], self.ldh[i], self.H[i], self.ldh[i], self.XH[i],
                                    self.ldh[i], B, h, self.bpart[i], self.act, **self._pre_kw(i))
                    E = ops.col_moments_chunks(B)
                    sums, dbeta = self.bpart[i], lay.view(g, 'beta%d' % i)
                    if comm.dp:
                        sums, E = self._reduce_bwd_sums(i, E, h, dbeta), 1
                        dbeta = None
                    ops.bn_bwd_apply(self.dH[i], self.ldh[i], self.H[i], self.ldh[i], self.XH[i],
                                     self.ldh[i], self.inv_std[i], sums, E, float(Bg), B, h,
                                     self.dZ[i], self.ldh[i], dbeta, self.act, **self._pre_kw(i))
                else:
                    ops.relu_bwd(self.dH[i], self.ldh[i], self._slope_in(i), self.ldh[i], B, h, self.dZ[i],
                                 self.ldh[i], self.act)
            Kp = lay.G_in if i == 0 else lay.hidden[i - 1]
            gW = lay.view(g, 'W%d' % i)
            if i == 0:
                with self._t('gemm_enc0_dW'):
                    if self._sparse_dw(B):
                        if self.cc_in.lutp is None:
                            self._not_capturing('first use of the byte-store weight gradient')
                            self.cc_in.ensure_lut(ops)
                        ops.enc0_dw_sparse(self.cc_in, self._kperm, self._kcur, 0, B, Kp, h, self.dZ[0], self.ldh[0], gW, h,
                                           self.ws_enc0)
                    elif self._h2_enc0(B, True):
# ... 369 lines not shown
```

dca_amd/ops.py:

```python
import ctypes

import torch

from . import hip


class HipOps:
    name = 'hip'
    device_type = 'cuda'

    def __init__(self):
        hip.require_gpu()
        self.L = hip.lib()
        self.max_partials = self.L.dcahip_zinb_max_partials()

    def zinb_nll(self, a_mean, a_disp, a_pi, lda, theta_w, Y, ldy, sf, perm, cursor, B, G, ridge,
                 inv_n, flags, d_mean, d_disp, d_pi, ldd, partials):
        n = ctypes.c_int(0)
        p = hip.ptr
        hip.check(self.L.dcahip_zinb_nll(p(a_mean), p(a_disp), p(a_pi), lda, p(theta_w), p(Y), ldy,
                                         p(sf), p(perm), p(cursor), B, G, ridge, inv_n, flags,
                                         p(d_mean), p(d_disp), p(d_pi), ldd, p(partials),
                                         ctypes.byref(n), hip.stream()), 'zinb_nll')
        return n.value
# ... 27 lines not shown
        p = hip.ptr
        hip.check(self.L.dcahip_nll_marginals(p(a_mean), p(a_disp), p(a_pi), lda, p(theta_w), p(Y), ldy, p(sf), B, G,
                                              ridge, flags, p(cell_out), p(gene_acc), p(ws), hip.stream()), 'nll_marginals')

    def group_moments_workspace_doubles(self, B, G, K):
        n = int(self.L.dcahip_group_moments_workspace_doubles(B, G, K))
        hip.check(min(n, 0), 'group_moments_workspace_doubles')
        return n

    def group_moments(self, a_mean, lda, sf, codes, B, G, K, flags, sum_acc, sumsq_acc, ldg, ws):
        p = hip.ptr
        hip.check(self.L.dcahip_group_moments(p(a_mean), lda, p(sf), p(codes), B, G, K, flags, p(sum_acc), p(sumsq_acc),
                                              ldg, p(ws), hip.stream()), 'group_moments')

    def gram_workspace_doubles(self, B, G):
        n = int(self.L.dcahip_gram_workspace_doubles(B, G))
        hip.check(min(n, 0), 'gram_workspace_doubles')
        return n

    def gram(self, x, ldx, cols, keep, shift, B, G, cross, ldc, dsum, ws):
        p = hip.ptr
        hip.check(self.L.dcahip_gram(p(x), ldx, p(cols), p(keep), p(shift), B, G, p(cross), ldc, p(dsum), p(ws),
                                     hip.stream()), 'gram')

    def loss_finalize(self, partials, n, scale, loss_out):
        hip.check(self.L.dcahip_loss_finalize(hip.ptr(partials), n, scale, hip.ptr(loss_out),
                                              hip.stream()), 'loss_finalize')

    def step_end(self, loss, weight, hist, rows_per_slot, acc, cursor, advance):
        p = hip.ptr
        hip.check(self.L.dcahip_step_end(p(loss), weight, p(hist), rows_per_slot, p(acc), p(cursor),
                                         advance, hip.stream()), 'step_end')

    def heads_infer(self, a_mean, a_disp, a_pi, lda, sf, B, G, mean_sf, theta, pi, ldo, flags=0):
        p = hip.ptr
        hip.check(self.L.dcahip_zinb_heads_infer(p(a_mean), p(a_disp), p(a_pi), lda, p(sf), B, G,
                                                 p(mean_sf), p(theta), p(pi), ldo, flags, hip.stream()),
                  'heads_infer')

    def heads_fused_workspace_bytes(self, B, hL, G, plane, flags):
        return self.L.dcahip_heads_fused_workspace_bytes(B, hL, G, plane, flags)

    def x3_product_32x32(self, A, B, C, K):
        hip.check(self.L.dcahip_x3_product_32x32(hip.ptr(A), hip.ptr(B), hip.ptr(C), K, hip.stream()), "x3_product_32x32")

    def has(self, entry):
        return hasattr(self.L, entry)

    def heads_tile_order_len(self, G):
        return int(self.L.dcahip_heads_tile_order_len(G))

    def heads_fused(self, H, ldh, Wh, ldw, bh, plane, theta_w, Y, ldy, sf, perm, cursor, B, hL, G,
                    ridge, inv_n, flags, gW, ldg, g_theta, dH, lddh, partials, ws, tile_order=None, loss_out=None,
                    compact=None, d_exp=0):
        n = ctypes.c_int(0)
        p = hip.ptr
        c = compact
        hip.check(self.L.dcahip_heads_fused(p(H), ldh, p(Wh), ldw, p(bh), plane, p(theta_w), p(Y), ldy,
                                            p(c.Yc) if c is not None else None, c.ldc if c is not None else 0,
                                            p(c.ovf_ptr) if c is not None else None,
                                            p(c.ovf_col) if c is not None else None,
                                            p(c.ovf_val) if c is not None else None,
                                            p(sf), p(perm), p(cursor), B, hL, G, ridge, inv_n, flags,
                                            p(gW), ldg, p(g_theta), p(dH), lddh, p(partials),
                                            ctypes.byref(n), p(ws), ws.numel() * ws.element_size(),
                                            p(tile_order), p(loss_out), int(d_exp), hip.stream()), 'heads_fused')
        return n.value

    def counts_compact_ld(self, G):
        return int(self.L.dcahip_counts_compact_ld(G))

    def counts_compact(self, Y, ldy, n, G, Yc, ldc, status):
        hip.check(self.L.dcahip_counts_compact(hip.ptr(Y), ldy, n, G, hip.ptr(Yc), ldc, hip.ptr(status), hip.stream()),
                  'counts_compact')

    def enc0_lut_entries(self):
        return int(self.L.dcahip_enc0_lut_entries())

    def enc0_lut(self, fac, do_log, n, lutp):
        hip.check(self.L.dcahip_enc0_lut(hip.ptr(fac), int(do_log), n, hip.ptr(lutp), hip.stream()), 'enc0_lut')

    def enc0_sparse_supported(self, H1):
        return bool(self.L.dcahip_enc0_sparse_supported(int(H1)))

    def enc0_dw_sparse_workspace_bytes(self, B, G, H1):
        return int(self.L.dcahip_enc0_dw_sparse_workspace_bytes(B, G, H1))

    def enc0_dw_sparse(self, c, perm, cursor, row_base, B, G, H1, dZ, ldz, gW, ldg, ws, form=0):
        p = hip.ptr
        c.ensure_lut(self)
        hip.check(self.L.dcahip_enc0_dw_sparse(p(c.Yc), c.ldc, p(c.ovf_ptr), p(c.ovf_col), p(c.ovf_val), p(c.fac),
                                               int(c.do_log), p(c.lutp), p(c.mean), p(c.std), p(perm), p(cursor), int(row_base),
                                               B, G, H1, p(dZ), ldz, p(gW), ldg, p(ws), ws.numel() * ws.element_size(),
                                               int(form), hip.stream()), 'enc0_dw_sparse')

    def enc0_fwd_lut_workspace_bytes(self, B, G, H1):
        return int(self.L.dcahip_enc0_fwd_lut_workspace_bytes(B, G, H1))

    def enc0_fwd_lut(self, c, perm, cursor, row_base, B, G, H1, W, ldw, bias, Z, ldz, ws):
        p = hip.ptr
        c.ensure_lut(self)
        hip.check(self.L.dcahip_enc0_fwd_lut(p(c.Yc), c.ldc, p(c.ovf_ptr), p(c.ovf_col), p(c.ovf_val), p(c.fac),
                                             int(c.do_log), p(c.lutp), p(c.mean), p(c.std), p(perm), p(cursor), int(row_base),
                                             B, G, H1, p(W), ldw, p(bias), p(Z), ldz, p(ws),
                                             ws.numel() * ws.element_size(), hip.stream()), 'enc0_fwd_lut')

    def sgemm_workspace_bytes(self, ta, tb, M, N, K, colsum_row=False, split_k=0):
        return self.L.dcahip_sgemm_workspace_bytes(int(ta), int(tb), M, N, K, int(colsum_row), split_k)

    def sgemm(self, ta, tb, M, N, K, A, lda, B, ldb, C, ldc, bias=None, perm=None, cursor=None,
              colsum_row=False, split_k=0, ws=None):
        p = hip.ptr
        wsb = ws.numel() * ws.element_size() if ws is not None else 0
        hip.check(self.L.dcahip_sgemm(int(ta), int(tb), M, N, K, p(A), lda, p(B), ldb, p(C), ldc,
                                      p(bias), p(perm), p(cursor), int(colsum_row), split_k, p(ws),
                                      wsb, hip.stream()), 'sgemm')

    def sgemm_plan(self, ta, tb, M, N, K, A, lda, B, ldb, colsum_row=False, split_k=0):
        out = (ctypes.c_int * 8)()
        hip.check(self.L.dcahip_sgemm_plan(int(ta), int(tb), M, N, K, int(colsum_row), split_k, hip.ptr(A), lda,
                                           hip.ptr(B), ldb, ctypes.addressof(out)), 'sgemm_plan')
# ... 104 lines not shown
                                               momentum, eps, int(act), p(Z), ldz, p(xhat), ldx, p(Hout), ldh, p(inv_std),
                                               hip.stream()), 'dense_bn_small')

    def hidden_small_chain(self, layers, Hin, ldin, B, batchnorm, momentum, eps, act):
        arr = self._small_layers(layers)
        hip.check(self.L.dcahip_hidden_small_chain(arr, len(layers), hip.ptr(Hin), ldin, B, int(batchnorm), momentum, eps,
                                                   int(act), hip.stream()), 'hidden_small_chain')

    @property
    def hidden_stack_max_rows(self):
        return int(self.L.dcahip_hidden_stack_max_rows())

    def hidden_stack_workspace_bytes(self, n_layers, B):
        return int(self.L.dcahip_hidden_stack_workspace_bytes(n_layers, B))

    def hidden_stack_fwd(self, layers, B, momentum, eps, act, ws, rows_per_wg=64, steps=None):
        arr = self._small_layers(layers)
        first, last = steps if steps is not None else (0, len(layers))
        hip.check(self.L.dcahip_hidden_stack_fwd(arr, len(layers), B, momentum, eps, int(act), int(rows_per_wg), first, last,
                                                 hip.ptr(ws), ws.numel() * ws.element_size(), hip.stream()), 'hidden_stack_fwd')

    def hidden_stack_bwd(self, layers, B, n_total, act, dZ0, ldz0, ws, rows_per_wg=64, steps=None):
        arr = self._bwd_layers(layers)
        first, last = steps if steps is not None else (0, len(layers) + 1)
        hip.check(self.L.dcahip_hidden_stack_bwd(arr, len(layers), B, float(n_total), int(act), hip.ptr(dZ0), ldz0,
                                                 int(rows_per_wg), first, last, hip.ptr(ws),
                                                 0 if ws is None else ws.numel() * ws.element_size(),
                                                 hip.stream()), 'hidden_stack_bwd')

    def _small_layers(self, layers):
        arr = (hip.SmallLayer * len(layers))()
        for q, d in zip(arr, layers):
            for k in ('W', 'bias', 'beta', 'moving_mean', 'moving_var', 'Z', 'xhat', 'Hout', 'inv_std'):
                setattr(q, k, hip.ptr(d.get(k)))
            for k in ('ldw', 'K', 'H', 'ldz', 'ldx', 'ldh'):
                setattr(q, k, int(d.get(k, 0)))
        return arr

    def _bwd_layers(self, layers):
        arr = (hip.StackBwdLayer * len(layers))()
        for q, d in zip(arr, layers):
            for k in ('W', 'Hact', 'xhat', 'inv_std', 'Hprev', 'gW', 'dbeta', 'dH', 'beta'):
                setattr(q, k, hip.ptr(d.get(k)))
            for k in ('ldw', 'K', 'H', 'ldh', 'ldx', 'ldp', 'ldg', 'lddh'):
                setattr(q, k, int(d.get(k, 0)))
        return arr

    def hidden_stack_fwd_sync(self, layers, B, momentum, eps, act, step, ext_entries, ext_counts, ext_E, stat_out, ws):
        arr = self._small_layers(layers)
        hip.check(self.L.dcahip_hidden_stack_fwd_sync(arr, len(layers), B, momentum, eps, int(act), int(step),
                                                      hip.ptr(ext_entries), hip.ptr(ext_counts), int(ext_E), hip.ptr(stat_out),
                                                      hip.ptr(ws), ws.numel() * ws.element_size(), hip.stream()),
                  'hidden_stack_fwd_sync')

    def hidden_stack_bwd_sync(self, layers, B, n_total, act, dZ0, ldz0, step, ext_sums, sums_out, ws):
        arr = self._bwd_layers(layers)
        hip.check(self.L.dcahip_hidden_stack_bwd_sync(arr, len(layers), B, float(n_total), int(act), hip.ptr(dZ0), ldz0,
                                                      int(step), hip.ptr(ext_sums), hip.ptr(sums_out), hip.ptr(ws),
                                                      ws.numel() * ws.element_size(), hip.stream()), 'hidden_stack_bwd_sync')

    def dense_bn_bwd_small(self, dH, ldd, Hact, ldh, xhat, ldx, inv_std, Hp, ldp, W, ldw, B, K, H, batchnorm, n_total, act,
                           gW, ldg, dbeta, dHp, lddp, beta=None):
        p = hip.ptr
        hip.check(self.L.dcahip_dense_bn_bwd_small(p(dH), ldd, p(Hact), ldh, p(xhat), ldx, p(inv_std), p(Hp), ldp, p(W), ldw,
                                                   B, K, H, int(batchnorm), float(n_total), int(act), p(gW), ldg, p(dbeta),
                                                   p(dHp), lddp, p(beta), hip.stream()), 'dense_bn_bwd_small')

    def relu_bwd(self, dH, ldd, Hact, ldh, B, H, dZ, ldz, act=1):
        p = hip.ptr
        hip.check(self.L.dcahip_relu_bwd(p(dH), ldd, p(Hact), ldh, B, H, p(dZ), ldz, act, hip.stream()),
                  'relu_bwd')

    def relu_fwd(self, Z, ldz, B, H, Hout, ldh, act=1):
        hip.check(self.L.dcahip_relu_fwd(hip.ptr(Z), ldz, B, H, hip.ptr(Hout), ldh, act, hip.stream()),
                  'relu_fwd')

    def colsum_chain(self, x, ldx, B, N, theta_w, out):
        p = hip.ptr
        hip.check(self.L.dcahip_colsum_chain(p(x), ldx, B, N, p(theta_w), p(out), hip.stream()),
                  'colsum_chain')

    def optimizer_step(self, kind, w, g, slot1, slot2, n, lr, it, clip):
        p = hip.ptr
        hip.check(self.L.dcahip_optimizer_step(hip.OPT_KINDS[kind], p(w), p(g), p(slot1), p(slot2), n, p(lr),
                                               p(it), clip, hip.stream()), 'optimizer_step')

    def prelu_workspace_doubles(self, h):
        return int(self.L.dcahip_prelu_workspace_doubles(h))

    def prelu_fwd(self, x, ldx, alpha, B, h, out, ldo):
        p = hip.ptr
        hip.check(self.L.dcahip_prelu_fwd(p(x), ldx, p(alpha), B, h, p(out), ldo, hip.stream()), 'prelu_fwd')

    def prelu_bwd(self, d, ldd, x, ldx, alpha, B, h, galpha, ws):
        p = hip.ptr
        hip.check(self.L.dcahip_prelu_bwd(p(d), ldd, p(x), ldx, p(alpha), B, h, p(galpha), p(ws), hip.stream()),
                  'prelu_bwd')

    def elempi_workspace_doubles(self, G):
        return int(self.L.dcahip_elempi_workspace_doubles(G))

    def elempi_fwd(self, a_mean, lda, k, c, B, G, a_pi, ldp):
        p = hip.ptr
        hip.check(self.L.dcahip_elempi_fwd(p(a_mean), lda, p(k), p(c), B, G, p(a_pi), ldp, hip.stream()), 'elempi_fwd')

    def elempi_bwd(self, m, lda, d_mean, d_pi, ldd, k, B, G, gk, gc, ws):
# ... 274 lines not shown
        r = dict(s=torch.full((n,), nan, dtype=torch.float64, device=dev), a=torch.full((n,), nan, dtype=torch.float64, device=dev),
                 b=torch.full((n,), nan, dtype=torch.float64, device=dev), nearest=torch.full((n,), -1, dtype=torch.int32, device=dev),
                 counts=torch.zeros(k, dtype=torch.int32, device=dev),
                 cluster_mean=torch.full((k,), nan, dtype=torch.float64, device=dev),
                 mean=torch.full((1,), nan, dtype=torch.float64, device=dev))
        status = torch.zeros(1, dtype=torch.int32, device=dev)
        hip.check(self.L.dcahip_silhouette(p(X) if n else None, ldx, n, d, p(labels) if n else None, k, splits, p(r['s']), p(r['a']),
                                           p(r['b']), p(r['nearest']), p(r['counts']), p(r['cluster_mean']), p(r['mean']),
                                           p(ws), p(status), hip.stream()), 'silhouette')
        self.silhouette_raise(status, r['counts'])
        return r

    def csr_gather(self, csr, perm, cursor, row0, B, sf, fac, do_log, mean, std, Y, ldy, X, ldx, sf_out, status):
        p = hip.ptr
        hip.check(self.L.dcahip_csr_gather(p(csr.indptr), p(csr.indices), p(csr.values), csr.nnz, csr.n, csr.G, p(perm),
                                           p(cursor), int(row0), B, p(sf), p(fac), int(bool(do_log)), p(mean), p(std),
                                           p(Y), ldy, p(X), ldx if X is not None else 0, p(sf_out), p(status),
                                           hip.stream()), 'csr_gather')

    def csr_gather_cols(self, csr, col_out, G_out, perm, cursor, row0, B, sf, fac, do_log, mean, std, Y, ldy, X, ldx, sf_out,
                        status):
        p = hip.ptr
        assert col_out.dtype == torch.int32 and col_out.numel() >= csr.G
        hip.check(self.L.dcahip_csr_gather_cols(p(csr.indptr), p(csr.indices), p(csr.values), csr.nnz, csr.n, csr.G, p(perm),
                                                p(cursor), int(row0), B, p(sf), p(fac), int(bool(do_log)), p(mean), p(std),
                                                p(Y), ldy, p(X), ldx if X is not None else 0, p(sf_out), p(status),
                                                p(col_out), int(G_out), hip.stream()), 'csr_gather_cols')

    def csr_gather_compact(self, csr, perm, cursor, row0, B, sf, fac, do_log, mean, std, Yc, ldc, ovf_ptr, ovf_col, ovf_val,
                           X, ldx, sf_out, fac_out, status):
        p = hip.ptr
        cap = int(ovf_col.numel()) if ovf_col is not None else 0
        hip.check(self.L.dcahip_csr_gather_compact(p(csr.indptr), p(csr.indices), p(csr.values), csr.nnz, csr.n, csr.G,
                                                   p(perm), p(cursor), int(row0), B, p(sf), p(fac), int(bool(do_log)), p(mean),
                                                   p(std), p(Yc), ldc, p(ovf_ptr), p(ovf_col), p(ovf_val), cap, p(X),
                                                   ldx if X is not None else 0, p(sf_out), p(fac_out), p(status),
                                                   hip.stream()), 'csr_gather_compact')

    def csr_col_pass(self, csr, fac, do_log, col_part, status):
        p = hip.ptr
        hip.check(self.L.dcahip_csr_col_pass(p(csr.indptr), p(csr.indices), p(csr.values), csr.nnz, csr.n, csr.G, p(fac),
                                             int(bool(do_log)), p(col_part), p(status), hip.stream()), 'csr_col_pass')

    def csr_row_sums(self, csr, out, status):
        p = hip.ptr
        hip.check(self.L.dcahip_csr_row_sums(p(csr.indptr), p(csr.indices), p(csr.values), csr.nnz, csr.n, csr.G, p(out),
                                             p(status), hip.stream()), 'csr_row_sums')

    def rmsprop_clip_end(self, w, g, ms, n, lr, rho, eps, clip, loss, weight, hist, rows_per_slot, acc, cursor, advance):
        p = hip.ptr
        hip.check(self.L.dcahip_rmsprop_clip(p(w), p(g), p(ms), n, p(lr), rho, eps, clip, p(loss), weight, p(hist),
                                             rows_per_slot, p(acc), p(cursor), advance, hip.stream()), 'rmsprop_clip')

    def rmsprop_clip(self, w, g, ms, n, lr, rho, eps, clip):
        self.rmsprop_clip_end(w, g, ms, n, lr, rho, eps, clip, None, 0.0, None, 0, None, None, 0)
```

include/dcahip.h:

```cpp
#ifndef DCAHIP_H
#define DCAHIP_H

#ifdef __cplusplus
extern "C" {
#endif

#define DCAHIP_VERSION 2
#define DCAHIP_EINVAL (-22)

#define DCAHIP_NLL_HAS_PI      1
#define DCAHIP_NLL_CONST_DISP  2
#define DCAHIP_NLL_POISSON     4
#define DCAHIP_NLL_MSE         8

int dcahip_version(void);

int dcahip_zinb_max_partials(void);

int dcahip_zinb_nll(const float* a_mean, const float* a_disp, const float* a_pi, long lda,
                    const float* theta_w,
                    const float* y, long ldy, const float* sf,
                    const int* perm, const long long* cursor,
                    int B, int G, float ridge, float inv_n, int flags,
                    float* d_mean, float* d_disp, float* d_pi, long ldd,
// ... 5 lines not shown
                           float inv_n, int flags, void* d_planes, long ldp, long plane_stride,
                           long col_mean, long col_disp, long col_pi, float* d_theta, long ldd_theta,
                           double* loss_partials, int* n_partials_out, void* stream);

int dcahip_zinb_nll_planes_h2(const float* a_mean, const float* a_disp, const float* a_pi, long lda,
                              const float* theta_w, const float* y, long ldy, const float* sf,
                              const int* perm, const long long* cursor, int B, int G, float ridge,
                              float inv_n, int flags, int d_exp, void* d_planes, long ldp, long plane_stride,
                              long col_mean, long col_disp, long col_pi, float* d_theta, long ldd_theta,
                              double* loss_partials, int* n_partials_out, void* stream);

int dcahip_nll_marginals_workspace_doubles(int B, int G);
int dcahip_nll_marginals(const float* a_mean, const float* a_disp, const float* a_pi, long lda,
                         const float* theta_w, const float* y, long ldy, const float* sf,
                         int B, int G, float ridge, int flags,
                         double* cell_out, double* gene_acc, double* workspace, void* stream);

#define DCAHIP_GROUP_NO_SF   16
#define DCAHIP_GROUP_LOG1P   32
int dcahip_group_moments_workspace_doubles(int B, int G, int K);
int dcahip_group_moments(const float* a_mean, long lda, const float* sf, const int* codes,
                         int B, int G, int K, int flags,
                         double* sum_acc, double* sumsq_acc, long ldg,
                         double* workspace, void* stream);

long dcahip_gram_workspace_doubles(int B, int G);
int dcahip_gram(const float* x, long ldx, const int* cols, const int* keep, const double* shift,
                int B, int G, double* cross, long ldc, double* dsum, double* ws, void* stream);

int dcahip_loss_finalize(const double* partials, int n_partials, double scale,
                         float* loss_out, void* stream);

int dcahip_step_end(const float* loss, double weight, float* hist, int rows_per_slot,
                    double* acc, long long* cursor, int advance, void* stream);

int dcahip_zinb_heads_infer(const float* a_mean, const float* a_disp, const float* a_pi,
                            long lda, const float* sf, int B, int G,
                            float* mean_sf, float* theta, float* pi, long ldo, int flags,
                            void* stream);

long dcahip_heads_fused_workspace_bytes(int B, int hL, int G, long plane, int flags);
int dcahip_heads_tile_order_len(int G);
int dcahip_heads_fused(const float* H, long ldh, const float* Wh, long ldw, const float* bh,
                       long plane, const float* theta_w,
                       const float* y, long ldy,
                       const unsigned char* yc, long ldc, const int* ovf_ptr, const int* ovf_col,
                       const float* ovf_val, const float* sf,
                       const int* perm, const long long* cursor,
                       int B, int hL, int G, float ridge, float inv_n, int flags,
                       float* gW, long ldg, float* g_theta, float* dH, long lddh,
                       double* loss_partials, int* n_partials_out,
                       void* workspace, long workspace_bytes, const int* tile_order,
                       float* loss_out, int d_exp, void* stream);
int dcahip_x3_product_32x32(const float* A, const float* B, float* C, int K, void* stream);

int dcahip_sgemm(int ta, int tb, int M, int N, int K,
                 const float* A, long lda, const float* B, long ldb, float* C, long ldc,
                 const float* bias, const int* perm, const long long* cursor,
                 int colsum_row, int split_k, void* workspace, long workspace_bytes,
                 void* stream);
long dcahip_sgemm_workspace_bytes(int ta, int tb, int M, int N, int K, int colsum_row, int split_k);
int dcahip_sgemm_plan(int ta, int tb, int M, int N, int K, int colsum_row, int split_k,
                      const float* A, long lda, const float* B, long ldb, int out[8]);
int dcahip_split_planes(const float* src, long ld, const int* perm, const long long* cursor, long R, int C,
                        void* planes, long ldp, long plane_stride, void* stream);
int dcahip_gemm_p3(int ta, int tb, int M, int N, int K, const void* A, long lda, long plane_a,
                   const void* B, long ldb, long plane_b, float* C, long ldc, const float* bias,
                   const int* perm, const long long* cursor, int colsum_row, int split_k,
                   void* workspace, long workspace_bytes, void* stream);
long dcahip_gemm_p3_workspace_bytes(int M, int N, int K, int colsum_row, int split_k);
int dcahip_absmax_exp(const float* src, long ld, long R, int C, int* exp_out, void* scratch_word, void* stream);
int dcahip_split_planes_h2(const float* src, long ld, const int* perm, const long long* cursor, long R, int C,
                           void* planes, long ldp, long plane_stride, const int* exp, void* stream);
int dcahip_gemm_h2_supported(int M, int N, int K);
long dcahip_gemm_h2_workspace_bytes(int M, int N, int K, int colsum_row, int split_k);
int dcahip_gemm_h2(int ta, int tb, int M, int N, int K, const void* A, long lda, long plane_a, const int* exp_a, int exp_a_add,
                   const void* B, long ldb, long plane_b, const int* exp_b, int exp_b_add, float alpha,
                   float* C, long ldc, const float* bias, int colsum_row, int split_k,
                   void* workspace, long workspace_bytes, void* stream);
int dcahip_transpose(const float* src, long ld_src, int R, int C, float* dst, long ld_dst, void* stream);
int dcahip_transpose_rows(const float* src, long ld_src, const int* perm, const long long* cursor, int R, int C,
                          float* dst, long ld_dst, void* stream);

int dcahip_col_moments_chunks(int B);
int dcahip_col_moments(const float* Z, long ldz, int B, int H, float* part, void* stream);
int dcahip_moments_combine(const float* entries, const float* counts, int E, int H,
                           float* out , void* stream);
int dcahip_bn_relu_apply(const float* Z, long ldz, int B, int H,
                         const float* entries, const float* counts, int E,
                         const float* beta, float* moving_mean, float* moving_var,
                         float momentum, float eps, int relu,
                         float* Hout, long ldh, float* xhat, long ldx, float* inv_std,
                         void* stream);

int dcahip_bn_fused_max_rows(void);
int dcahip_dense_small_max_k(void);
int dcahip_dense_bn_small(const float* Hp, long ldp, const float* W, long ldw, const float* bias,
                          int B, int K, int H, int batchnorm, const float* beta,
                          float* moving_mean, float* moving_var, float momentum, float eps, int act,
                          float* Z, long ldz, float* xhat, long ldx, float* Hout, long ldh,
                          float* inv_std, void* stream);
int dcahip_dense_bn_bwd_small(const float* dH, long ldd, const float* Hact, long ldh,
                              const float* xhat, long ldx, const float* inv_std,
                              const float* Hp, long ldp, const float* W, long ldw,
                              int B, int K, int H, int batchnorm, float n_total, int act,
                              float* gW, long ldg, float* dbeta, float* dHp, long lddp, const float* beta,
                              void* stream);
typedef struct dcahip_small_layer {
    const float* W; long ldw;
    const float* bias;
    int K, H;
    const float* beta; float* moving_mean; float* moving_var;
    float* Z; long ldz;
    float* xhat; long ldx; float* Hout; long ldh; float* inv_std;
} dcahip_small_layer;
int dcahip_hidden_small_chain(const dcahip_small_layer* layers, int n, const float* Hin, long ldin, int B,
                              int batchnorm, float momentum, float eps, int act, void* stream);
typedef struct dcahip_stack_bwd_layer {
    const float* W; long ldw; int K, H;
    const float* Hact; long ldh;
    const float* xhat; long ldx; const float* inv_std;
    const float* Hprev; long ldp;
    float* gW; long ldg; float* dbeta;
    float* dH; long lddh;
    const float* beta;
} dcahip_stack_bwd_layer;
int dcahip_hidden_stack_max_rows(void);
long dcahip_hidden_stack_workspace_bytes(int n_layers, int B);
int dcahip_hidden_stack_fwd(const dcahip_small_layer* layers, int n, int B, float momentum, float eps, int act,
                            int rows_per_wg, int first_step, int last_step,
                            void* workspace, long workspace_bytes, void* stream);
int dcahip_hidden_stack_bwd(const dcahip_stack_bwd_layer* layers, int n, int B, float n_total, int act,
                            float* dZ0, long ldz0, int rows_per_wg, int first_step, int last_step,
                            void* workspace, long workspace_bytes, void* stream);

int dcahip_hidden_stack_step_blocks(int B);
int dcahip_hidden_stack_fwd_sync(const dcahip_small_layer* layers, int n, int B, float momentum, float eps, int act,
                                 int step, const float* ext_entries, const float* ext_counts, int ext_E,
                                 float* stat_out, void* workspace, long workspace_bytes, void* stream);
int dcahip_hidden_stack_bwd_sync(const dcahip_stack_bwd_layer* layers, int n, int B, float n_total, int act,
                                 float* dZ0, long ldz0, int step, const float* ext_sums, float* sums_out,
                                 void* workspace, long workspace_bytes, void* stream);
int dcahip_bn_relu_train_small(const float* Z, long ldz, int B, int H, const float* beta,
                               float* moving_mean, float* moving_var, float momentum, float eps,
                               int act, float* Hout, long ldh, float* xhat, long ldx,
                               float* inv_std, void* stream);
int dcahip_bn_bwd_small(const float* dH, long ldd, const float* Hact, long ldh,
                        const float* xhat, long ldx, const float* inv_std, float n_total,
                        int B, int H, float* dZ, long ldz, float* dbeta, int act, const float* beta, void* stream);

int dcahip_bn_bwd_sums(const float* dH, long ldd, const float* Hact, long ldh,
                       const float* xhat, long ldx, int B, int H, float* part, int act, const float* beta,
                       void* stream);
int dcahip_bn_bwd_apply(const float* dH, long ldd, const float* Hact, long ldh,
                        const float* xhat, long ldx, const float* inv_std,
                        const float* sums, int E, float n_total, int B, int H,
                        float* dZ, long ldz, float* dbeta, int act, const float* beta, void* stream);
int dcahip_relu_bwd(const float* dH, long ldd, const float* Hact, long ldh, int B, int H,
                    float* dZ, long ldz, int act, void* stream);
int dcahip_relu_fwd(const float* Z, long ldz, int B, int H, float* Hout, long ldh, int act, void* stream);
int dcahip_prelu_workspace_doubles(int h);
int dcahip_prelu_fwd(const float* x, long ldx, const float* alpha, int B, int h, float* out, long ldo, void* stream);
int dcahip_prelu_bwd(float* d, long ldd, const float* x, long ldx, const float* alpha, int B, int h,
                     float* galpha, double* workspace, void* stream);
int dcahip_elempi_workspace_doubles(int G);
int dcahip_elempi_fwd(float* a_mean, long lda, const float* k, const float* c, int B, int G,
                      float* a_pi, long ldp, void* stream);
int dcahip_elempi_bwd(const float* m, long lda, float* d_mean, const float* d_pi, long ldd, const float* k,
                      int B, int G, float* gk, float* gc, double* workspace, void* stream);
int dcahip_bcast_cols(const float* s, long lds, int B, int G, float* out, long ldo, void* stream);
int dcahip_row_sums_strided(const float* x, long ldx, int B, int G, float* out, long ldo, void* stream);

int dcahip_colsum_chain(const float* x, long ldx, int B, int N, const float* theta_w,
                        float* out, void* stream);

int dcahip_prep_chunks(int n);
int dcahip_prep_row_sums(const float* Y, long ldy, int n, int G, float* out, void* stream);
int dcahip_prep_col_pass(const float* Y, long ldy, int n, int G, const float* fac, int do_log,
                         float* X, long ldx, double* col_part, void* stream);
int dcahip_prep_col_finish(const double* col_part, int R, int G, double n_total,
                           float* sums, float* mean, float* stdv, void* stream);
int dcahip_prep_scale(float* X, long ldx, int n, int G, const float* mean, const float* stdv,
                      void* stream);
int dcahip_csr_expand(const int* indptr, const int* indices, const float* values, long nnz, int rows, int G,
                      float* Y, long ldy, int* status, void* stream);

int dcahip_csr_compress(const float* X, long ld, int rows, int G, long base, long* indptr, int* indices, float* values,
                        long cap, int* status, void* stream);
int dcahip_csr_subset(const long* indptr, const int* indices, const float* values, long nnz, int n, int G,
                      const unsigned char* row_keep, const unsigned char* col_keep, int n_out, long* out_indptr,
                      int* out_indices, float* out_values, long cap, int* ws, int* status, void* stream);

int dcahip_csr_gather(const long* indptr, const int* indices, const float* values, long nnz, int n, int G,
                      const int* perm, const long long* cursor, long row0, int B, const float* sf,
                      const float* fac, int do_log, const float* mean, const float* stdv, float* Y, long ldy,
                      float* X, long ldx, float* sf_out, int* status, void* stream);
int dcahip_csr_gather_cols(const long* indptr, const int* indices, const float* values, long nnz, int n, int G,
                           const int* perm, const long long* cursor, long row0, int B, const float* sf,
                           const float* fac, int do_log, const float* mean, const float* stdv, float* Y, long ldy,
                           float* X, long ldx, float* sf_out, int* status, const int* col_out, int G_out, void* stream);
int dcahip_csr_gather_compact(const long* indptr, const int* indices, const float* values, long nnz, int n, int G,
                              const int* perm, const long long* cursor, long row0, int B, const float* sf,
                              const float* fac, int do_log, const float* mean, const float* stdv,
                              unsigned char* Yc, long ldc, int* ovf_ptr, int* ovf_col, float* ovf_val, int ovf_cap,
                              float* X, long ldx, float* sf_out, float* fac_out, int* status, void* stream);
int dcahip_csr_col_pass(const long* indptr, const int* indices, const float* values, long nnz, int n, int G,
                        const float* fac, int do_log, double* col_part, int* status, void* stream);
int dcahip_csr_row_sums(const long* indptr, const int* indices, const float* values, long nnz, int n, int G,
                        float* out, int* status, void* stream);

long dcahip_csr_thin_workspace_bytes(int n, long nnz);
int dcahip_csr_thin(const long* indptr, const int* indices, const float* values, long nnz, int n, int G,
                    const long* row_ids, unsigned long long threshold, unsigned long long seed,
                    long* indptr_a, int* indices_a, float* values_a,
                    long* indptr_b, int* indices_b, float* values_b, long cap,
                    void* workspace, int* status, void* stream);

int dcahip_rmsprop_clip(float* w, const float* g, float* ms, long n, const float* lr,
                        float rho, float eps, float clip, const float* loss, double weight,
                        float* hist, int rows_per_slot, double* acc, long long* cursor, int advance,
                        void* stream);

#define DCAHIP_OPT_SGD       0
#define DCAHIP_OPT_RMSPROP   1
#define DCAHIP_OPT_ADAGRAD   2
#define DCAHIP_OPT_ADADELTA  3
#define DCAHIP_OPT_ADAM      4
#define DCAHIP_OPT_ADAMAX    5
int dcahip_optimizer_step(int kind, float* w, const float* g, float* slot1, float* slot2, long n,
                          const float* lr, const long long* iter, float clip, void* stream);
int dcahip_counter_add(long long* counter, int v, void* stream);
int dcahip_nadam_step(float* w, const float* g, float* m, float* v, long n, const float* lr,
                      const long long* iter, float* m_schedule, float clip, void* stream);
#define DCAHIP_REG_MAX_SEGS 16
typedef struct {
    int nseg;
    long start[DCAHIP_REG_MAX_SEGS];
    long end[DCAHIP_REG_MAX_SEGS];
    float l1[DCAHIP_REG_MAX_SEGS];
    float l2[DCAHIP_REG_MAX_SEGS];
} dcahip_reg_desc;
int dcahip_l1l2_workspace_doubles(void);
int dcahip_l1l2_apply(const dcahip_reg_desc* d, const float* w, float* g, float* loss_inout,
                      double* workspace, void* stream);

int dcahip_dropout_apply(const float* x, long ldx, const int* perm, const long long* cursor, int B, int h,
                         float rate, unsigned long long seed, const long long* step, int layer, long row0,
                         float* out, long ldo, void* stream);

long dcahip_counts_compact_ld(int G);
int dcahip_counts_compact(const float* Y, long ldy, int n, int G, unsigned char* Yc, long ldc, int* status,
                          void* stream);
int dcahip_enc0_sparse_supported(int H1);
int dcahip_enc0_lut(const float* fac, int do_log, int n, void* lutp, void* stream);
int dcahip_enc0_lut_entries(void);
long dcahip_enc0_dw_sparse_workspace_bytes(int B, int G, int H1);
int dcahip_enc0_dw_sparse(const unsigned char* Yc, long ldc, const int* ovf_ptr, const int* ovf_col,
                          const float* ovf_val, const float* fac, int do_log, const void* lutp, const float* mean,
                          const float* stdv, const int* perm, const long long* cursor, long row_base,
                          int B, int G, int H1, const float* dZ, long ldz, float* gW, long ldg,
                          void* workspace, long workspace_bytes, int form, void* stream);
long dcahip_enc0_fwd_lut_workspace_bytes(int B, int G, int H1);
int dcahip_enc0_fwd_lut(const unsigned char* Yc, long ldc, const int* ovf_ptr, const int* ovf_col,
                        const float* ovf_val, const float* fac, int do_log, const void* lutp, const float* mean,
                        const float* stdv, const int* perm, const long long* cursor, long row_base,
                        int B, int G, int H1, const float* W, long ldw, const float* bias,
                        float* Z, long ldz, void* workspace, long workspace_bytes, void* stream);

int dcahip_knn_splits(int nq, int n, int d, int k);
long dcahip_knn_workspace_bytes(int nq, int n, int d, int k, int splits);
int dcahip_knn(const float* Q, long ldq, int nq, const float* X, long ldx, int n, int d, int k,
               long self_offset, int splits, int* idx_out, float* d2_out, long ldo,
               void* ws, int* status, void* stream);

// ... 24 lines not shown
```

Before: 4.572 million.

## Fuse heads dW reduction and RMSprop update into hidden-stack backward steps

The heads dW partial reduction, previously a separate kernel, is deferred. It now runs in slices as extra 'rider' workgroups launched alongside each hidden-stack backward step. Those riders also apply the RMSprop update to the heads weights directly, and the global optimizer kernel skips those weight ranges. The goal is to hide the bandwidth-heavy dW reduce and its update behind the latency-bound small-layer backward steps, and to drop one pass over the large heads gradient. The cost is more complex scheduling, a risk of contention with the stack kernels, and extra validation paths.

```diff
diff --git a/dca_amd/build.py b/dca_amd/build.py
--- a/dca_amd/build.py
+++ b/dca_amd/build.py
@@ -10,7 +10,7 @@
 SOURCES = ['dcahip_zinb.hip', 'dcahip_gemm.hip', 'dcahip_layers.hip', 'dcahip_heads.hip', 'dcahip_prep.hip', 'dcahip_opt.hip',
            'dcahip_dropout.hip', 'dcahip_sparse.hip', 'dcahip_peer.hip', 'dcahip_knn.hip', 'dcahip_kmeans.hip', 'dcahip_gram.hip',
            'dcahip_silhouette.hip']
-HEADERS = ['zinb_math.hpp', 'h2_math.hpp', 'philox.hpp', 'knn_dist.hpp']
+HEADERS = ['zinb_math.hpp', 'h2_math.hpp', 'philox.hpp', 'knn_dist.hpp', 'heads_dw_reduce.hpp']
 ARCH = 'gfx950'
 HOST_LIB = os.path.join(CSRC, 'libdcahost.so')
 HOST_SOURCES = ['dcahost_tsv.cpp', 'dcahost_read.cpp']
diff --git a/dca_amd/config.py b/dca_amd/config.py
--- a/dca_amd/config.py
+++ b/dca_amd/config.py
@@ -20,16 +20,18 @@
     fused_write: bool = True
     resident: str = 'auto'
     counts_compact: bool = False
+    heads_update_ride: bool = True
     graph_steps: int = 8
     sparse_dw_min: int = 512
     lut_fwd_min: int = 1024
     enc0_nt_min: int = 256
     predict_chunk: int = 1024
+    heads_ride_workgroups: int = 256
 
     _ENV = {'stack': 'DCA_AMD_STACK', 'bwd_chain': 'DCA_AMD_BWD_CHAIN', 'wide_planes': 'DCA_AMD_WIDE_PLANES', 'wide_h2': 'DCA_AMD_WIDE_H2',
             'dp_sharded_opt': 'DCA_AMD_DP_SHARDED_OPT', 'dp_graph': 'DCA_AMD_DP_GRAPH', 'device_prep': 'DCA_AMD_DEVICE_PREP',
             'fused_write': 'DCA_AMD_FUSED_WRITE', 'dp_peer_exchange': 'DCA_AMD_DP_PEER', 'resident': 'DCA_AMD_RESIDENT',
-            'counts_compact': 'DCA_AMD_COUNTS_COMPACT'}
+            'counts_compact': 'DCA_AMD_COUNTS_COMPACT', 'heads_update_ride': 'DCA_AMD_HEADS_RIDE'}
 
     @classmethod
     def from_env(cls):
diff --git a/dca_amd/csrc/dcahip_heads.hip b/dca_amd/csrc/dcahip_heads.hip
--- a/dca_amd/csrc/dcahip_heads.hip
+++ b/dca_amd/csrc/dcahip_heads.hip
@@ -3,6 +3,7 @@
 #include <type_traits>
 #include "dcahip.h"
 #include "zinb_math.hpp"
+#include "heads_dw_reduce.hpp"
 
 namespace {
 
@@ -820,69 +821,13 @@
 }
 
 
-struct ReduceDwArgs {
-    const float* ws; int S; long stride; int hL; long ldws, ncols; float* gW; long ldg;
-    const float* theta_w; float* g_theta; int G;
-    float scale;
-    const float* ws2; int S2; const int* tail_tiles; int ntail; long plane;
-    int tail_first;
-};
-
-__device__ __forceinline__ void reduce_dw_body(const ReduceDwArgs& q, int bid, int nblk) {
-    const int hL = q.hL;
-    const long ldws = q.ldws, ncols = q.ncols; float* gW = q.gW; const long ldg = q.ldg;
-    const float* theta_w = q.theta_w; float* g_theta = q.g_theta; const int G = q.G;
-    const float sc = q.scale;
-    __shared__ unsigned tailbm[kMaxGrid / 32];
-    if (q.ntail > 0) {
-        for (int i = threadIdx.x; i < kMaxGrid / 32; i += 256) tailbm[i] = 0u;
-        __syncthreads();
-        for (int i = threadIdx.x; i < q.ntail; i += 256) {
-            const int tl = q.tail_tiles ? q.tail_tiles[i] : q.tail_first + i;
-            if (tl >= 0 && tl < kMaxGrid) atomicOr(&tailbm[tl >> 5], 1u << (tl & 31));
-        }
-        __syncthreads();
-    }
-    auto is_tail = [&](long col_in_plane) { const int tl = (int)(col_in_plane / kTG); return q.ntail > 0 && ((tailbm[tl >> 5] >> (tl & 31)) & 1u); };
-    if ((ncols & 3) == 0 && (ldws & 3) == 0 && (ldg & 3) == 0 && (q.stride & 3) == 0 && (q.plane & 3) == 0 &&
-        ((reinterpret_cast<uintptr_t>(q.ws) | reinterpret_cast<uintptr_t>(gW) | reinterpret_cast<uintptr_t>(q.ws2)) & 15) == 0) {
-        const long nq = ncols >> 2, totalq = (long)(hL + 1) * nq;
-        for (long idx = (long)bid * 256 + threadIdx.x; idx < totalq; idx += (long)nblk * 256) {
-            const long i = idx / nq, c = (idx - i * nq) << 2;
-            const bool tl = is_tail(c % q.plane);
-            const float* ws = tl ? q.ws2 : q.ws; const int S = tl ? q.S2 : q.S; const long stride = q.stride;
-            float4 v = *reinterpret_cast<const float4*>(ws + i * ldws + c);
-            for (int s = 1; s < S; ++s) {
-                const float4 x = *reinterpret_cast<const float4*>(ws + (long)s * stride + i * ldws + c);
-                v.x += x.x; v.y += x.y; v.z += x.z; v.w += x.w;
-            }
-            v.x *= sc; v.y *= sc; v.z *= sc; v.w *= sc;
-            *reinterpret_cast<float4*>(gW + i * ldg + c) = v;
-        }
-    } else {
-        const long total = (long)(hL + 1) * ncols;
-        for (long idx = (long)bid * 256 + threadIdx.x; idx < total; idx += (long)nblk * 256) {
-            const long i = idx / ncols, c = idx - i * ncols;
-            const bool tl = is_tail(c % q.plane);
-            const float* ws = tl ? q.ws2 : q.ws; const int S = tl ? q.S2 : q.S;
-            float v = 0.f;
-            for (int s = 0; s < S; ++s) v += ws[(long)s * q.stride + i * ldws + c];
-            gW[i * ldg + c] = v * sc;
-        }
-    }
-    if (g_theta) {
-        for (long c = (long)bid * 256 + threadIdx.x; c < G; c += (long)nblk * 256) {
-            const bool tl = is_tail(c);
-            const float* ws = tl ? q.ws2 : q.ws; const int S = tl ? q.S2 : q.S; const long stride = q.stride;
-            float v = 0.f;
-            for (int s = 0; s < S; ++s) v += ws[(long)s * stride + (long)(hL + 1) * ldws + c];
-            const float e = expf(theta_w[c]);
-            g_theta[c] = (e >= 1e-3f && e <= 1e4f) ? v * sc * e : 0.f;
-        }
-    }
-}
-
-__global__ __launch_bounds__(256) void heads_reduce_dw_kernel(ReduceDwArgs q) { reduce_dw_body(q, blockIdx.x, gridDim.x); }
+static_assert(kDwMaxTiles == kMaxGrid && kDwTileGenes == kTG, "heads_dw_reduce.hpp keeps the tile constants of K-HEADS");
+
+__global__ __launch_bounds__(256) void heads_reduce_dw_kernel(ReduceDwArgs q) { reduce_dw_body<false, 1>(q, DwUpdate{}, blockIdx.x, gridDim.x, 0, 1); }
+
+__global__ __launch_bounds__(256) void heads_dw_update_kernel(ReduceDwArgs q, DwUpdate u, int slice, int nslices) {
+    reduce_dw_body<true, 4>(q, u, blockIdx.x, gridDim.x, slice, nslices);
+}
 
 struct ReduceDhArgs {
     const float* ws; int ntg, B, Bpad, KT, hL; float* dH; long lddh; float scale;
@@ -962,7 +907,7 @@
 template <int GL>
 __global__ __launch_bounds__(256) void heads_reduce_both_kernel(ReduceDhArgs qh, ReduceDwArgs qw, int n_dh) {
     if ((int)blockIdx.x < n_dh) reduce_dh_body<GL>(qh, blockIdx.x);
-    else reduce_dw_body(qw, blockIdx.x - n_dh, gridDim.x - n_dh);
+    else reduce_dw_body<false, 1>(qw, DwUpdate{}, blockIdx.x - n_dh, gridDim.x - n_dh, 0, 1);
 }
 
 
@@ -1510,19 +1455,51 @@
 
 extern "C" int dcahip_heads_tile_order_len(int G) { return G > 0 ? (((G + kTG - 1) / kTG + kWG - 1) / kWG) * kWG : 0; }
 
-extern "C" int dcahip_heads_fused(const float* H, long ldh, const float* Wh, long ldw,
-                                  const float* bh, long plane, const float* theta_w,
-                                  const float* y, long ldy,
-                                  const unsigned char* yc, long ldc, const int* ovf_ptr, const int* ovf_col,
-                                  const float* ovf_val, const float* sf, const int* perm,
-                                  const long long* cursor, int B, int hL, int G, float ridge,
-                                  float inv_n, int flags, float* gW, long ldg, float* g_theta,
-                                  float* dH, long lddh, double* loss_partials, int* n_partials_out,
-                                  void* workspace, long workspace_bytes, const int* tile_order,
-                                  float* loss_out, int d_exp, void* stream) {
+static ReduceDwArgs dw_reduce_args(const HeadsPlan& pl, int hL, int G, long plane, bool cdisp, float* gW, long ldg,
+                                   const float* theta_w, float* g_theta, float inv_n, void* workspace, const int* tile_order) {
+    float* ws_dh = static_cast<float*>(workspace);
+    float* ws_dw = ws_dh + pl.dh_bytes / sizeof(float);
+    float* ws_dh2 = ws_dw + pl.dw_bytes / sizeof(float);
+    float* ws_dw2 = ws_dh2 + pl.dh2_bytes / sizeof(float);
+    return ReduceDwArgs{ws_dw, pl.S, pl.dw_stride, hL, pl.ldws, pl.ldws, gW, ldg, cdisp ? theta_w : nullptr,
+                        cdisp ? g_theta : nullptr, G, inv_n,
+                        ws_dw2, pl.S2, (pl.ntail > 0 && tile_order) ? tile_order + pl.nmain : nullptr, pl.ntail, plane, pl.nmain};
+}
+
+bool heads_dw_reduce_args(int B, int hL, int G, long plane, int flags, float* gW, long ldg, const float* theta_w,
+                          float* g_theta, float inv_n, void* workspace, long workspace_bytes, const int* tile_order,
+                          ReduceDwArgs* out) {
+    const bool has_pi = flags & DCAHIP_NLL_HAS_PI, cdisp = flags & DCAHIP_NLL_CONST_DISP;
+    HeadsPlan pl;
+    if (!make_heads_plan(B, hL, G, plane, flags, &pl) || pl.S < 2) return false;
+    if (!gW || !workspace || !al16(workspace) || (cdisp && (!theta_w || !g_theta))) return false;
+    if (workspace_bytes < pl.dw_bytes + pl.dh_bytes + pl.hs_bytes + pl.dw2_bytes + pl.dh2_bytes) return false;
+    const int NH = 1 + (cdisp ? 0 : 1) + (has_pi ? 1 : 0);
+    if (ldg < (long)NH * plane) return false;
+    *out = dw_reduce_args(pl, hL, G, plane, cdisp, gW, ldg, theta_w, g_theta, inv_n, workspace, tile_order);
+    return true;
+}
+
+extern "C" int dcahip_heads_fused_dw_partials(int B, int hL, int G, long plane, int flags) {
+    HeadsPlan pl;
+    if (!make_heads_plan(B, hL, G, plane, flags, &pl)) return 0;
+    return pl.S;
+}
+
+static int heads_fused_launch(const float* H, long ldh, const float* Wh, long ldw,
+                              const float* bh, long plane, const float* theta_w,
+                              const float* y, long ldy,
+                              const unsigned char* yc, long ldc, const int* ovf_ptr, const int* ovf_col,
+                              const float* ovf_val, const float* sf, const int* perm,
+                              const long long* cursor, int B, int hL, int G, float ridge,
+                              float inv_n, int flags, float* gW, long ldg, float* g_theta,
+                              float* dH, long lddh, double* loss_partials, int* n_partials_out,
+                              void* workspace, long workspace_bytes, const int* tile_order,
+                              float* loss_out, int d_exp, void* stream, bool defer_dw) {
     const bool has_pi = flags & DCAHIP_NLL_HAS_PI, cdisp = flags & DCAHIP_NLL_CONST_DISP;
     HeadsPlan pl;
     if (!make_heads_plan(B, hL, G, plane, flags, &pl)) return DCAHIP_EINVAL;
+    if (defer_dw && pl.S < 2) return DCAHIP_EINVAL;
     if (!H || !Wh || !bh || (!y && !yc) || !sf || !gW || !dH || !loss_partials || !workspace) return DCAHIP_EINVAL;
     if (cdisp && (!theta_w || !g_theta)) return DCAHIP_EINVAL;
     if (workspace_bytes < pl.dw_bytes + pl.dh_bytes + pl.hs_bytes + pl.dw2_bytes + pl.dh2_bytes) return DCAHIP_EINVAL;
@@ -1588,12 +1565,10 @@
         long gr = (total / 4 + 255) / 256;
         if (gr > 2048) gr = 2048;
         if (gr < 1) gr = 1;
-        const ReduceDwArgs qw{ws_dw, pl.S, pl.dw_stride, hL, pl.ldws, pl.ldws, gW, ldg, cdisp ? theta_w : nullptr,
-                              cdisp ? g_theta : nullptr, G, inv_n,
-                              ws_dw2, pl.S2, (pl.ntail > 0 && tile_order) ? tile_order + pl.nmain : nullptr, pl.ntail, plane, pl.nmain};
+        const ReduceDwArgs qw = dw_reduce_args(pl, hL, G, plane, cdisp, gW, ldg, theta_w, g_theta, inv_n, workspace, tile_order);
         const int gl = (nq <= 1024 && pl.npart >= 256) ? 64 : (nq >= 64L * 512 ? 4 : 16);
         const int n_dh = (int)((nq + 256 / gl - 1) / (256 / gl));
-        if (!direct_dw) {
+        if (!direct_dw && !defer_dw) {
             const dim3 grid(n_dh + (int)gr);
             if (gl == 64) hipLaunchKernelGGL(heads_reduce_both_kernel<64>, grid, dim3(256), 0, s, qh, qw, n_dh);
             else if (gl == 4) hipLaunchKernelGGL(heads_reduce_both_kernel<4>, grid, dim3(256), 0, s, qh, qw, n_dh);
@@ -1607,3 +1582,50 @@
     }
     return rc;
 }
+
+extern "C" int dcahip_heads_fused(const float* H, long ldh, const float* Wh, long ldw,
+                                  const float* bh, long plane, const float* theta_w,
+                                  const float* y, long ldy,
+                                  const unsigned char* yc, long ldc, const int* ovf_ptr, const int* ovf_col,
+                                  const float* ovf_val, const float* sf, const int* perm,
+                                  const long long* cursor, int B, int hL, int G, float ridge,
+                                  float inv_n, int flags, float* gW, long ldg, float* g_theta,
+                                  float* dH, long lddh, double* loss_partials, int* n_partials_out,
+                                  void* workspace, long workspace_bytes, const int* tile_order,
+                                  float* loss_out, int d_exp, void* stream) {
+    return heads_fused_launch(H, ldh, Wh, ldw, bh, plane, theta_w, y, ldy, yc, ldc, ovf_ptr, ovf_col, ovf_val, sf, perm, cursor,
+                              B, hL, G, ridge, inv_n, flags, gW, ldg, g_theta, dH, lddh, loss_partials, n_partials_out,
+                              workspace, workspace_bytes, tile_order, loss_out, d_exp, stream, false);
+}
+
+extern "C" int dcahip_heads_fused_dh(const float* H, long ldh, const float* Wh, long ldw,
+                                     const float* bh, long plane, const float* theta_w,
+                                     const float* y, long ldy,
+                                     const unsigned char* yc, long ldc, const int* ovf_ptr, const int* ovf_col,
+                                     const float* ovf_val, const float* sf, const int* perm,
+                                     const long long* cursor, int B, int hL, int G, float ridge,
+                                     float inv_n, int flags, float* gW, long ldg, float* g_theta,
+                                     float* dH, long lddh, double* loss_partials, int* n_partials_out,
+                                     void* workspace, long workspace_bytes, const int* tile_order,
+                                     float* loss_out, int d_exp, void* stream) {
+    return heads_fused_launch(H, ldh, Wh, ldw, bh, plane, theta_w, y, ldy, yc, ldc, ovf_ptr, ovf_col, ovf_val, sf, perm, cursor,
+                              B, hL, G, ridge, inv_n, flags, gW, ldg, g_theta, dH, lddh, loss_partials, n_partials_out,
+                              workspace, workspace_bytes, tile_order, loss_out, d_exp, stream, true);
+}
+
+extern "C" int dcahip_heads_dw_update(const float* ws, int S, long stride, int hL, long ldws, long ncols, float* gW, long ldg,
+                                      float* theta_w, float* g_theta, int G, float scale,
+                                      const float* ws2, int S2, const int* tail_tiles, int ntail, long plane, int tail_first,
+                                      float* w, float* ms, float* ms_theta, const float* lr, float rho, float eps, float clip,
+                                      int slice, int nslices, int workgroups, void* stream) {
+    if (!ws || S < 1 || hL < 0 || ncols <= 0 || ldws < ncols || ldg < ncols || !gW || !w || !ms || !lr) return DCAHIP_EINVAL;
+    if (plane <= 0 || (g_theta && (!theta_w || !ms_theta || G <= 0 || G > plane || G > ldws))) return DCAHIP_EINVAL;
+    if (stride < (long)(hL + (g_theta ? 2 : 1)) * ldws) return DCAHIP_EINVAL;
+    if (ntail < 0 || (ntail > 0 && (!ws2 || S2 < 1)) || (plane + kTG - 1) / kTG > kMaxGrid) return DCAHIP_EINVAL;
+    if (nslices < 1 || slice < 0 || slice >= nslices || workgroups < 1 || workgroups > 2048) return DCAHIP_EINVAL;
+    const ReduceDwArgs q{ws, S, stride, hL, ldws, ncols, gW, ldg, g_theta ? theta_w : nullptr, g_theta, G, scale,
+                         ws2, S2, tail_tiles, ntail, plane, tail_first};
+    const DwUpdate u{w, ms, theta_w, ms_theta, lr, rho, eps, clip};
+    hipLaunchKernelGGL(heads_dw_update_kernel, dim3(workgroups), dim3(256), 0, static_cast<hipStream_t>(stream), q, u, slice, nslices);
+    return (int)hipGetLastError();
+}
diff --git a/dca_amd/csrc/dcahip_layers.hip b/dca_amd/csrc/dcahip_layers.hip
--- a/dca_amd/csrc/dcahip_layers.hip
+++ b/dca_amd/csrc/dcahip_layers.hip
@@ -1,6 +1,7 @@
 #include <hip/hip_runtime.h>
 #include <stdint.h>
 #include "dcahip.h"
+#include "heads_dw_reduce.hpp"
 
 namespace {
 
@@ -902,9 +903,7 @@
     const float* loss; double weight; float* hist; int rows_per_slot; double* acc; long long* cursor; int advance; int on;
 };
 
-__global__ __launch_bounds__(256) void rmsprop_clip_kernel(float* w, const float* g, float* ms,
-                                                           long n, const float* lrp, float rho,
-                                                           float eps, float clip, StepEnd se) {
+__device__ __forceinline__ void step_end_apply(const StepEnd& se) {
     if (se.on && blockIdx.x == 0 && threadIdx.x == 0) {
         const long long c = se.cursor ? *se.cursor : 0;
         if (se.loss) {
@@ -914,30 +913,57 @@
         }
         if (se.cursor) *se.cursor = c + se.advance;
     }
-    const float lr = *lrp;
+}
+
+template <bool TAIL_FMA>
+__device__ __forceinline__ void rmsprop_clip_span(float* w, const float* g, float* ms, long n, float lr, float rho, float eps,
+                                                  float clip, int bid, int nblk) {
+    const float omr = 1.f - rho;
     const long nv = n >> 2;
-    const long stride = (long)gridDim.x * 256;
-    for (long i = (long)blockIdx.x * 256 + threadIdx.x; i < nv; i += stride) {
+    const long stride = (long)nblk * 256;
+    for (long i = (long)bid * 256 + threadIdx.x; i < nv; i += stride) {
         float4 gv = reinterpret_cast<const float4*>(g)[i];
         float4 mv = reinterpret_cast<const float4*>(ms)[i];
         float4 wv = reinterpret_cast<const float4*>(w)[i];
         float* gp = &gv.x; float* mp = &mv.x; float* wp = &wv.x;
 #pragma unroll
-        for (int j = 0; j < 4; ++j) {
-            float gj = gp[j];
-            if (clip > 0.f) gj = fminf(fmaxf(gj, -clip), clip);
-            mp[j] = rho * mp[j] + (1.f - rho) * gj * gj;
-            wp[j] = wp[j] - lr * gj / (sqrtf(mp[j]) + eps);
-        }
+        for (int j = 0; j < 4; ++j) rmsprop_clip_elem<true>(gp[j], mp[j], wp[j], lr, rho, omr, eps, clip);
         reinterpret_cast<float4*>(ms)[i] = mv;
         reinterpret_cast<float4*>(w)[i] = wv;
     }
-    for (long i = (nv << 2) + (long)blockIdx.x * 256 + threadIdx.x; i < n; i += stride) {
-        float gj = g[i];
-        if (clip > 0.f) gj = fminf(fmaxf(gj, -clip), clip);
-        const float m = rho * ms[i] + (1.f - rho) * gj * gj;
+    for (long i = (nv << 2) + (long)bid * 256 + threadIdx.x; i < n; i += stride) {
+        float m = ms[i], wi = w[i];
+        rmsprop_clip_elem<TAIL_FMA>(g[i], m, wi, lr, rho, omr, eps, clip);
         ms[i] = m;
-        w[i] = w[i] - lr * gj / (sqrtf(m) + eps);
+        w[i] = wi;
+    }
+}
+
+__global__ __launch_bounds__(256) void rmsprop_clip_kernel(float* w, const float* g, float* ms,
+                                                           long n, const float* lrp, float rho,
+                                                           float eps, float clip, StepEnd se) {
+    step_end_apply(se);
+    rmsprop_clip_span<false>(w, g, ms, n, *lrp, rho, eps, clip, blockIdx.x, gridDim.x);
+}
+
+struct KeepRanges { long lo[3], hi[3]; };
+
+__global__ __launch_bounds__(256) void rmsprop_clip_skip_kernel(float* w, const float* g, float* ms, KeepRanges kr,
+                                                                const float* lrp, float rho, float eps, float clip, StepEnd se) {
+    step_end_apply(se);
+    const float lr = *lrp, omr = 1.f - rho;
+#pragma unroll
+    for (int r = 0; r < 3; ++r) {
+        const long lo = kr.lo[r], hi = kr.hi[r];
+        if (hi <= lo) continue;
+        const long a = min((lo + 3) & ~3L, hi);
+        for (long i = lo + (long)blockIdx.x * 256 + threadIdx.x; i < a; i += (long)gridDim.x * 256) {
+            float m = ms[i], wi = w[i];
+            rmsprop_clip_elem<true>(g[i], m, wi, lr, rho, omr, eps, clip);
+            ms[i] = m;
+            w[i] = wi;
+        }
+        rmsprop_clip_span<true>(w + a, g + a, ms + a, hi - a, lr, rho, eps, clip, blockIdx.x, gridDim.x);
     }
 }
 
@@ -1220,6 +1246,40 @@
     if (nbar) grid_exit(a.sync, (unsigned)nwg);
 }
 
+__device__ __forceinline__ void stack_gw_sum(const StackBwdArgs& a, const int wg, float* smf) {
+    const int tid = threadIdx.x, nwg = a.nwg;
+    for (int i = 1; i < a.n; ++i) {
+        const StackBwdLayer& L = a.l[i];
+        const int total = (L.K + 1) * L.H;
+        const float* gw = a.gwp + (long)i * nwg * 65 * 64;
+        const int el = tid & 31, sl = tid >> 5;
+        const int per = (nwg + 7) / 8;
+        for (int e0 = wg * 32; e0 < total; e0 += nwg * 32) {
+            const int e = e0 + el;
+            const int ec = e < total ? e : total - 1;
+            const int k = ec / L.H, cc = ec - k * L.H;
+            const float* src = gw + (long)k * 64 + cc;
+            float v = 0.f;
+            for (int b0 = sl * per; b0 < min(nwg, (sl + 1) * per); b0 += 16) {
+                float pv[16];
+#pragma unroll
+                for (int u = 0; u < 16; ++u) pv[u] = src[(long)min(b0 + u, nwg - 1) * 65 * 64];
+#pragma unroll
+                for (int u = 0; u < 16; ++u) if (b0 + u < min(nwg, (sl + 1) * per)) v += pv[u];
+            }
+            __syncthreads();
+            smf[tid] = v;
+            __syncthreads();
+            if (tid < 32 && e < total) {
+                float t = 0.f;
+#pragma unroll
+                for (int q8 = 0; q8 < 8; ++q8) t += smf[q8 * 32 + tid];
+                L.gW[(long)k * L.ldg + cc] = t;
+            }
+        }
+    }
+}
+
 __global__ __launch_bounds__(256) void hidden_stack_bwd_kernel(StackBwdArgs a) {
     __shared__ __attribute__((aligned(16))) float dyt[kStackRows * kStackLd];
     __shared__ __attribute__((aligned(16))) float xt[kStackRows * kStackLd];
@@ -1360,38 +1420,15 @@
     }
     if (a.last > a.n) {
         if (fresh) grid_barrier(a.sync, (unsigned)nwg * (++nbar));
-        for (int i = 1; i < a.n; ++i) {
-            const StackBwdLayer& L = a.l[i];
-            const int total = (L.K + 1) * L.H;
-            const float* gw = a.gwp + (long)i * nwg * 65 * 64;
-            const int el = tid & 31, sl = tid >> 5;
-            const int per = (nwg + 7) / 8;
-            for (int e0 = wg * 32; e0 < total; e0 += nwg * 32) {
-                const int e = e0 + el;
-                const int ec = e < total ? e : total - 1;
-                const int k = ec / L.H, cc = ec - k * L.H;
-                const float* src = gw + (long)k * 64 + cc;
-                float v = 0.f;
-                for (int b0 = sl * per; b0 < min(nwg, (sl + 1) * per); b0 += 16) {
-                    float pv[16];
-#pragma unroll
-                    for (int u = 0; u < 16; ++u) pv[u] = src[(long)min(b0 + u, nwg - 1) * 65 * 64];
-#pragma unroll
-                    for (int u = 0; u < 16; ++u) if (b0 + u < min(nwg, (sl + 1) * per)) v += pv[u];
-                }
-                __syncthreads();
-                smf[tid] = v;
-                __syncthreads();
-                if (tid < 32 && e < total) {
-                    float t = 0.f;
-#pragma unroll
-                    for (int q8 = 0; q8 < 8; ++q8) t += smf[q8 * 32 + tid];
-                    L.gW[(long)k * L.ldg + cc] = t;
-                }
-            }
-        }
+        stack_gw_sum(a, wg, smf);
     }
     if (nbar) grid_exit(a.sync, (unsigned)nwg);
+}
+
+__global__ __launch_bounds__(256) void stack_bwd_gw_ride_kernel(StackBwdArgs a, ReduceDwArgs q, DwUpdate u, int slice, int nslices) {
+    __shared__ float smf[256];
+    if ((int)blockIdx.x < a.nwg) stack_gw_sum(a, blockIdx.x, smf);
+    else reduce_dw_body<true, 4>(q, u, blockIdx.x - a.nwg, gridDim.x - a.nwg, slice, nslices);
 }
 
 __device__ __forceinline__ bool w_tile_vec(const float* W, long ldw, int H) {
@@ -1573,13 +1610,13 @@
     const float* ext_in;
 };
 
-__global__ __launch_bounds__(256) void stack_bwd_step_kernel(StepBwdArgs a) {
+__device__ __forceinline__ void stack_bwd_step_body(const StepBwdArgs& a, const int wg) {
     __shared__ __attribute__((aligned(16))) float dyt[kStepRows * kStackLd];
     __shared__ __attribute__((aligned(16))) float ht[kStepRows * kStackLd];
     __shared__ __attribute__((aligned(16))) float wl[64 * kStackLd];
     __shared__ float smf[256];
     const int tid = threadIdx.x, tx = tid & 63, ty = tid >> 6;
-    const int wg = blockIdx.x, E = a.nwg;
+    const int E = a.nwg;
     const int cr = chunk_rows(a.B, E);
     const int r0 = wg * cr;
     const int nrows = max(0, min(a.B, r0 + cr) - r0);
@@ -1696,6 +1733,13 @@
     }
     const float t1 = wg_rowlane_sum(s1, smf), t2 = wg_rowlane_sum(s2, smf);
     if (tx < K && ty == 0) { a.part_out[((long)wg * 2 + 0) * K + tx] = t1; a.part_out[((long)wg * 2 + 1) * K + tx] = t2; }
+}
+
+__global__ __launch_bounds__(256) void stack_bwd_step_kernel(StepBwdArgs a) { stack_bwd_step_body(a, blockIdx.x); }
+
+__global__ __launch_bounds__(256) void stack_bwd_step_ride_kernel(StepBwdArgs a, ReduceDwArgs q, DwUpdate u, int slice, int nslices) {
+    if ((int)blockIdx.x < a.nwg) stack_bwd_step_body(a, blockIdx.x);
+    else reduce_dw_body<true, 4>(q, u, blockIdx.x - a.nwg, gridDim.x - a.nwg, slice, nslices);
 }
 
 struct ChainBwdArgs {
@@ -2177,6 +2221,25 @@
     if (grid < 1) grid = 1;
     hipLaunchKernelGGL(rmsprop_clip_kernel, dim3((int)grid), dim3(256), 0,
                        static_cast<hipStream_t>(stream), w, g, ms, n, lr, rho, eps, clip,
+                       StepEnd{loss, weight, hist, rows_per_slot, acc, cursor, advance, (loss || hist || acc || cursor) ? 1 : 0});
+    return (int)hipGetLastError();
+}
+
+extern "C" int dcahip_rmsprop_clip_skip(float* w, const float* g, float* ms, long n, long skip0_lo, long skip0_hi,
+                                        long skip1_lo, long skip1_hi, const float* lr,
+                                        float rho, float eps, float clip, const float* loss, double weight,
+                                        float* hist, int rows_per_slot, double* acc, long long* cursor, int advance,
+                                        void* stream) {
+    if (!w || !g || !ms || !lr || n <= 0 || (n & 3)) return DCAHIP_EINVAL;
+    if (!al16(w) || !al16(g) || !al16(ms)) return DCAHIP_EINVAL;
+    if (skip0_lo < 0 || skip0_hi < skip0_lo || skip1_lo < skip0_hi || skip1_hi < skip1_lo || skip1_hi > n) return DCAHIP_EINVAL;
+    const KeepRanges kr{{0, skip0_hi, skip1_hi}, {skip0_lo, skip1_lo, n}};
+    const long kept = n - (skip0_hi - skip0_lo) - (skip1_hi - skip1_lo);
+    long grid = ((kept >> 2) + 255) / 256;
+    if (grid > 2048) grid = 2048;
+    if (grid < 1) grid = 1;
+    hipLaunchKernelGGL(rmsprop_clip_skip_kernel, dim3((int)grid), dim3(256), 0,
+                       static_cast<hipStream_t>(stream), w, g, ms, kr, lr, rho, eps, clip,
                        StepEnd{loss, weight, hist, rows_per_slot, acc, cursor, advance, (loss || hist || acc || cursor) ? 1 : 0});
     return (int)hipGetLastError();
 }
@@ -2355,3 +2418,38 @@
     hipLaunchKernelGGL(hidden_stack_bwd_kernel, dim3(a.nwg), dim3(256), 0, static_cast<hipStream_t>(stream), a);
     return (int)hipGetLastError();
 }
+
+extern "C" int dcahip_hidden_stack_bwd_ride(const dcahip_stack_bwd_layer* layers, int n, int B, float n_total, int act,
+                                            float* dZ0, long ldz0, int step, void* workspace, long workspace_bytes,
+                                            int hL, int G, long plane, int flags, float* gW, long ldg,
+                                            float* theta_w, float* g_theta, float inv_n,
+                                            void* heads_workspace, long heads_workspace_bytes, const int* tile_order,
+                                            float* w, float* ms, float* ms_theta, const float* lr, float rho, float eps,
+                                            float clip, int slice, int nslices, int rider_workgroups, void* stream) {
+    if (!stack_shape_ok(layers, n, B) || !dZ0 || !stack_workspace_ok(workspace, workspace_bytes, n, B)) return DCAHIP_EINVAL;
+    if (step < 0 || step > n + 1 || nslices < 1 || slice < 0 || slice >= nslices) return DCAHIP_EINVAL;
+    if (rider_workgroups < 1 || rider_workgroups > 1024 || !w || !ms || !lr) return DCAHIP_EINVAL;
+    StackBwdArgs a{};
+    if (stack_plan(n, B, kStepRows, step, step, n + 2, &a.nwg)) return DCAHIP_EINVAL;
+    if (!stack_bwd_layers(layers, n, act, true, a.l)) return DCAHIP_EINVAL;
+    ReduceDwArgs q;
+    if (!heads_dw_reduce_args(B, hL, G, plane, flags, gW, ldg, theta_w, g_theta, inv_n, heads_workspace, heads_workspace_bytes,
+                              tile_order, &q))
+        return DCAHIP_EINVAL;
+    if (q.g_theta && !ms_theta) return DCAHIP_EINVAL;
+    const DwUpdate u{w, ms, theta_w, ms_theta, lr, rho, eps, clip};
+    a.n = n; a.B = B; a.act = act; a.first = step; a.last = step; a.n_total = n_total;
+    a.dZ0 = dZ0; a.ldz0 = ldz0;
+    a.sync = static_cast<unsigned*>(workspace);
+    a.part = reinterpret_cast<float*>(static_cast<char*>(workspace) + 256);
+    a.gwp = a.part + (long)n * a.nwg * 2 * 64;
+    const dim3 grid(a.nwg + rider_workgroups);
+    hipStream_t st = static_cast<hipStream_t>(stream);
+    if (step <= n) {
+        const StepBwdArgs sq = stack_bwd_step(a.l, n, B, n_total, act, dZ0, ldz0, step, a.nwg, a.part);
+        hipLaunchKernelGGL(stack_bwd_step_ride_kernel, grid, dim3(256), 0, st, sq, q, u, slice, nslices);
+    } else {
+        hipLaunchKernelGGL(stack_bwd_gw_ride_kernel, grid, dim3(256), 0, st, a, q, u, slice, nslices);
+    }
+    return (int)hipGetLastError();
+}
diff --git a/dca_amd/csrc/heads_dw_reduce.hpp b/dca_amd/csrc/heads_dw_reduce.hpp
--- /dev/null
+++ b/dca_amd/csrc/heads_dw_reduce.hpp
@@ -0,0 +1,146 @@
+#pragma once
+#include <hip/hip_runtime.h>
+#include <stdint.h>
+
+constexpr int kDwMaxTiles = 2048;
+constexpr int kDwTileGenes = 32;
+
+template <bool FMA>
+__device__ __forceinline__ void rmsprop_clip_elem(float gj, float& m, float& w, float lr, float rho, float omr, float eps,
+                                                  float clip) {
+    if (clip > 0.f) gj = fminf(fmaxf(gj, -clip), clip);
+    const float t = __fmul_rn(__fmul_rn(omr, gj), gj);
+    m = FMA ? fmaf(rho, m, t) : __fadd_rn(__fmul_rn(rho, m), t);
+    w = __fsub_rn(w, __fdiv_rn(__fmul_rn(lr, gj), __fadd_rn(sqrtf(m), eps)));
+}
+
+struct ReduceDwArgs {
+    const float* ws; int S; long stride; int hL; long ldws, ncols; float* gW; long ldg;
+    const float* theta_w; float* g_theta; int G;
+    float scale;
+    const float* ws2; int S2; const int* tail_tiles; int ntail; long plane;
+    int tail_first;
+};
+
+struct DwUpdate {
+    float* w; float* ms; float* w_theta; float* ms_theta;
+    const float* lr; float rho, eps, clip;
+};
+
+template <bool UPD, int U>
+__device__ __forceinline__ void reduce_dw_body(const ReduceDwArgs& q, const DwUpdate& up, int bid, int nblk, int slice,
+                                               int nslices) {
+    const int hL = q.hL;
+    const long ldws = q.ldws, ncols = q.ncols; float* gW = q.gW; const long ldg = q.ldg;
+    const float* theta_w = q.theta_w; float* g_theta = q.g_theta; const int G = q.G;
+    const float sc = q.scale;
+    float lr = 0.f, omr = 0.f;
+    if (UPD) { lr = *up.lr; omr = 1.f - up.rho; }
+    __shared__ unsigned tailbm[kDwMaxTiles / 32];
+    if (q.ntail > 0) {
+        for (int i = threadIdx.x; i < kDwMaxTiles / 32; i += 256) tailbm[i] = 0u;
+        __syncthreads();
+        for (int i = threadIdx.x; i < q.ntail; i += 256) {
+            const int tl = q.tail_tiles ? q.tail_tiles[i] : q.tail_first + i;
+            if (tl >= 0 && tl < kDwMaxTiles) atomicOr(&tailbm[tl >> 5], 1u << (tl & 31));
+        }
+        __syncthreads();
+    }
+    auto is_tail = [&](long col_in_plane) { const int tl = (int)(col_in_plane / kDwTileGenes); return q.ntail > 0 && ((tailbm[tl >> 5] >> (tl & 31)) & 1u); };
+    if ((ncols & 3) == 0 && (ldws & 3) == 0 && (ldg & 3) == 0 && (q.stride & 3) == 0 && (q.plane & 3) == 0 &&
+        ((reinterpret_cast<uintptr_t>(q.ws) | reinterpret_cast<uintptr_t>(gW) | reinterpret_cast<uintptr_t>(q.ws2)) & 15) == 0 &&
+        (!UPD || ((reinterpret_cast<uintptr_t>(up.w) | reinterpret_cast<uintptr_t>(up.ms)) & 15) == 0)) {
+        const long nq = ncols >> 2, totalq = (long)(hL + 1) * nq;
+        const long lo = totalq * slice / nslices, hi = totalq * (slice + 1) / nslices;
+        const long step = (long)nblk * 256;
+        const bool flat = U > 1 && ldws == ncols && ldg == ncols && q.ntail == 0;
+        for (long idx0 = lo + (long)bid * 256 + threadIdx.x; idx0 < hi; idx0 += step * U) {
+            const float* src[U]; int S[U]; long off[U]; float4 v[U], mv[U], wv[U];
+#pragma unroll
+            for (int u = 0; u < U; ++u) {
+                const long idx = idx0 + u * step;
+                if (idx < hi) {
+                    if (flat) {
+                        src[u] = q.ws + (idx << 2); S[u] = q.S; off[u] = idx << 2;
+                    } else {
+                        const long i = idx / nq, c = (idx - i * nq) << 2;
+                        const bool tl = is_tail(c % q.plane);
+                        src[u] = (tl ? q.ws2 : q.ws) + i * ldws + c; S[u] = tl ? q.S2 : q.S; off[u] = i * ldg + c;
+                    }
+                    v[u] = *reinterpret_cast<const float4*>(src[u]);
+                    if (UPD) {
+                        mv[u] = *reinterpret_cast<const float4*>(up.ms + off[u]);
+                        wv[u] = *reinterpret_cast<const float4*>(up.w + off[u]);
+                    }
+                } else {
+                    S[u] = 0;
+                }
+            }
+            int smax = 0;
+#pragma unroll
+            for (int u = 0; u < U; ++u) smax = S[u] > smax ? S[u] : smax;
+            for (int s = 1; s < smax; ++s) {
+                float4 x[U];
+#pragma unroll
+                for (int u = 0; u < U; ++u) if (s < S[u]) x[u] = *reinterpret_cast<const float4*>(src[u] + (long)s * q.stride);
+#pragma unroll
+                for (int u = 0; u < U; ++u) if (s < S[u]) { v[u].x += x[u].x; v[u].y += x[u].y; v[u].z += x[u].z; v[u].w += x[u].w; }
+            }
+#pragma unroll
+            for (int u = 0; u < U; ++u) {
+                if (S[u] == 0) continue;
+                v[u].x *= sc; v[u].y *= sc; v[u].z *= sc; v[u].w *= sc;
+                *reinterpret_cast<float4*>(gW + off[u]) = v[u];
+                if (UPD) {
+                    rmsprop_clip_elem<true>(v[u].x, mv[u].x, wv[u].x, lr, up.rho, omr, up.eps, up.clip);
+                    rmsprop_clip_elem<true>(v[u].y, mv[u].y, wv[u].y, lr, up.rho, omr, up.eps, up.clip);
+                    rmsprop_clip_elem<true>(v[u].z, mv[u].z, wv[u].z, lr, up.rho, omr, up.eps, up.clip);
+                    rmsprop_clip_elem<true>(v[u].w, mv[u].w, wv[u].w, lr, up.rho, omr, up.eps, up.clip);
+                    *reinterpret_cast<float4*>(up.ms + off[u]) = mv[u];
+                    *reinterpret_cast<float4*>(up.w + off[u]) = wv[u];
+                }
+            }
+        }
+    } else {
+        const long total = (long)(hL + 1) * ncols;
+        const long lo = total * slice / nslices, hi = total * (slice + 1) / nslices;
+        for (long idx = lo + (long)bid * 256 + threadIdx.x; idx < hi; idx += (long)nblk * 256) {
+            const long i = idx / ncols, c = idx - i * ncols;
+            const bool tl = is_tail(c % q.plane);
+            const float* ws = tl ? q.ws2 : q.ws; const int S = tl ? q.S2 : q.S;
+            float v = 0.f;
+            for (int s = 0; s < S; ++s) v += ws[(long)s * q.stride + i * ldws + c];
+            v = v * sc;
+            gW[i * ldg + c] = v;
+            if (UPD) {
+                float m = up.ms[i * ldg + c], w = up.w[i * ldg + c];
+                rmsprop_clip_elem<true>(v, m, w, lr, up.rho, omr, up.eps, up.clip);
+                up.ms[i * ldg + c] = m;
+                up.w[i * ldg + c] = w;
+            }
+        }
+    }
+    if (g_theta) {
+        const long lo = (long)G * slice / nslices, hi = (long)G * (slice + 1) / nslices;
+        for (long c = lo + (long)bid * 256 + threadIdx.x; c < hi; c += (long)nblk * 256) {
+            const bool tl = is_tail(c);
+            const float* ws = tl ? q.ws2 : q.ws; const int S = tl ? q.S2 : q.S; const long stride = q.stride;
+            float v = 0.f;
+            for (int s = 0; s < S; ++s) v += ws[(long)s * stride + (long)(hL + 1) * ldws + c];
+            float w = theta_w[c];
+            const float e = expf(w);
+            const float gt = (e >= 1e-3f && e <= 1e4f) ? v * sc * e : 0.f;
+            g_theta[c] = gt;
+            if (UPD) {
+                float m = up.ms_theta[c];
+                rmsprop_clip_elem<true>(gt, m, w, lr, up.rho, omr, up.eps, up.clip);
+                up.ms_theta[c] = m;
+                up.w_theta[c] = w;
+            }
+        }
+    }
+}
+
+__attribute__((visibility("hidden"))) bool heads_dw_reduce_args(int B, int hL, int G, long plane, int flags, float* gW, long ldg, const float* theta_w,
+                          float* g_theta, float inv_n, void* workspace, long workspace_bytes, const int* tile_order,
+                          ReduceDwArgs* out);
diff --git a/dca_amd/engine.py b/dca_amd/engine.py
--- a/dca_amd/engine.py
+++ b/dca_amd/engine.py
@@ -166,6 +166,19 @@
         raise NotImplementedError('init=%r is not implemented on the MI355X path (available: %s)'
                                   % (name, ', '.join(KERAS_INITIALIZERS)))
     return np.ascontiguousarray(w, dtype=np.float32)
+
+
+def heads_ride_slices(total, nslices):
+    return [(total * k // nslices, total * (k + 1) // nslices) for k in range(nslices)]
+
+
+def heads_ride_ranges(wh0, hL, NH, th0, G):
+    r0 = (wh0, wh0 + (hL + 1) * NH)
+    return r0, ((th0, th0 + G) if th0 is not None else (r0[1], r0[1]))
+
+
+def heads_ride_keep(P, skip0, skip1):
+    return [(lo, hi) for lo, hi in ((0, skip0[0]), (skip0[1], skip1[0]), (skip1[1], P)) if hi > lo]
 
 
 class ParamLayout:
@@ -337,6 +350,8 @@
         self._tile_lut = False
         self.ws_enc0 = self.ws_enc0l = None
         self.ws_stack = None
+        self._rode = False
+        self._ride_partials = {}
         self.stack_mode = self.cfg.stack
         self.sparse_dw_min = self.cfg.sparse_dw_min
 
@@ -1330,6 +1345,13 @@
         if self.reg is not None:
             ops.l1l2_apply(self.reg, w, g, g[lay.P:], self.reg_ws)
         fused_end = self.opt_kind == 'rmsprop' and not self.has_dropout and hasattr(ops, 'rmsprop_clip_end')
+        if fused_end and self._rode:
+            self._rode = False
+            with self._t('rmsprop_clip'):
+                skip0, skip1 = self._ride_skip()
+                ops.rmsprop_clip_skip_end(w, g, self.ms, lay.P, skip0, skip1, self.lr, RMS_RHO, RMS_EPS, self.clip, g[lay.P:],
+                                          float(Bg), self.hist, rows_per_slot or max(self.Bmax, 1), self.acc, self.cursor, B)
+            return
         if fused_end:
             with self._t('rmsprop_clip'):
                 ops.rmsprop_clip_end(w, g, self.ms, lay.P, self.lr, RMS_RHO, RMS_EPS, self.clip, g[lay.P:], float(Bg),
@@ -1384,8 +1406,27 @@
                 s = torch.zeros(2 * lay.hidden[i], dtype=torch.float32, device=self.dev)
                 self.comm.all_reduce_sum(s)
 
-    def heads_fused_launch(self, B, KL, inv_n):
+    def _heads_ride(self, B):
+        ops = self.ops
+        if not (self.cfg.heads_update_ride and B > 0 and self.ws_heads is not None and self.opt_kind == 'rmsprop'
+                and self.reg is None and not self.has_dropout and not self.comm.dp
+                and hasattr(ops, 'hidden_stack_bwd_ride') and hasattr(ops, 'rmsprop_clip_skip_end')):
+            return False
+        if self._stack_chain(B) or self._stack_sync(B) or not self._stack_coop(B) or self._stack_rows(B) != 32 \
+                or (self.stack_mode == 'coop' and B <= 256 * 64):
+            return False
+        S = self._ride_partials.get(B)
+        if S is None:
+            S = self._ride_partials[B] = ops.heads_fused_dw_partials(B, self.lay.hL, self.lay.G_out, self.lay.Gp, self.flags)
+        return S >= 2
+
+    def _ride_skip(self):
+        lay = self.lay
+        return heads_ride_ranges(lay.seg['Wh'][0], lay.hL, lay.NH, lay.seg['theta_w'][0] if lay.const_disp else None, lay.G_out)
+
+    def heads_fused_launch(self, B, KL, inv_n, defer_dw=False):
         lay, w, g = self.lay, self.w, self.g
+        kw = {'defer_dw': True} if defer_dw else {}
         self.ops.heads_fused(self._hl[0], self._hl[1], lay.view(w, 'Wh'), lay.NH,
                              lay.view(w, 'bh'), lay.Gp,
                              lay.view(w, 'theta_w') if lay.const_disp else None, self.Y,
@@ -1393,16 +1434,17 @@
                              self.ridge, inv_n, self.flags, lay.view(g, 'Wh'), lay.NH,
                              lay.view(g, 'theta_w') if lay.const_disp else None,
                              self._dhl, self._hl[1], self.partials, self.ws_heads,
-                             tile_order=self.tile_order, loss_out=g[lay.P:], **self._heads_compact())
+                             tile_order=self.tile_order, loss_out=g[lay.P:], **kw, **self._heads_compact())
 
     def _forward_backward(self, B, Bg, inv_n):
         lay, ops, comm = self.lay, self.ops, self.comm
         w, g = self.w, self.g
         KL = self._hidden_forward(B, ('perm',), True, self.counts_world)
         self._last_heads_args = (B, KL, inv_n)
+        ride = self._rode = self._heads_ride(B)
         if self.ws_heads is not None:
             with self._t('heads_fused'):
-                self.heads_fused_launch(B, KL, inv_n)
+                self.heads_fused_launch(B, KL, inv_n, defer_dw=ride)
         else:
             self._heads_backward_unfused(B, KL, inv_n)
         self._launch_heads_bucket()
@@ -1435,6 +1477,15 @@
                 ops.hidden_stack_bwd(layers, B, float(Bg), self.act, self.dZ[0], self.ldh[0], None, rows_per_wg=64)
             elif self.stack_mode == 'coop' and B <= 256 * 64:
                 ops.hidden_stack_bwd(layers, B, float(Bg), self.act, self.dZ[0], self.ldh[0], self.ws_stack, rows_per_wg=64)
+            elif ride:
+                cd = lay.const_disp
+                for st in range(L + 2):
+                    ops.hidden_stack_bwd_ride(layers, B, float(Bg), self.act, self.dZ[0], self.ldh[0], st, self.ws_stack,
+                                              KL, lay.G_out, lay.Gp, self.flags, lay.view(g, 'Wh'), lay.NH,
+                                              lay.view(w, 'theta_w') if cd else None, lay.view(g, 'theta_w') if cd else None,
+                                              inv_n, self.ws_heads, self.tile_order, lay.view(w, 'Wh'), lay.view(self.ms, 'Wh'),
+                                              lay.view(self.ms, 'theta_w') if cd else None, self.lr, RMS_RHO, RMS_EPS,
+                                              self.clip, L + 2, self.cfg.heads_ride_workgroups)
             else:
                 for st in range(L + 2):
                     ops.hidden_stack_bwd(layers, B, float(Bg), self.act, self.dZ[0], self.ldh[0], self.ws_stack,
diff --git a/dca_amd/ops.py b/dca_amd/ops.py
--- a/dca_amd/ops.py
+++ b/dca_amd/ops.py
@@ -103,11 +103,12 @@
 
     def heads_fused(self, H, ldh, Wh, ldw, bh, plane, theta_w, Y, ldy, sf, perm, cursor, B, hL, G,
                     ridge, inv_n, flags, gW, ldg, g_theta, dH, lddh, partials, ws, tile_order=None, loss_out=None,
-                    compact=None, d_exp=0):
+                    compact=None, d_exp=0, defer_dw=False):
         n = ctypes.c_int(0)
         p = hip.ptr
         c = compact
-        hip.check(self.L.dcahip_heads_fused(p(H), ldh, p(Wh), ldw, p(bh), plane, p(theta_w), p(Y), ldy,
+        fn = self.L.dcahip_heads_fused_dh if defer_dw else self.L.dcahip_heads_fused
+        hip.check(fn(p(H), ldh, p(Wh), ldw, p(bh), plane, p(theta_w), p(Y), ldy,
                                             p(c.Yc) if c is not None else None, c.ldc if c is not None else 0,
                                             p(c.ovf_ptr) if c is not None else None,
                                             p(c.ovf_col) if c is not None else None,
@@ -118,6 +119,17 @@
                                             p(tile_order), p(loss_out), int(d_exp), hip.stream()), 'heads_fused')
         return n.value
 
+    def heads_fused_dw_partials(self, B, hL, G, plane, flags):
+        return int(self.L.dcahip_heads_fused_dw_partials(B, hL, G, plane, flags))
+
+    def heads_dw_update(self, ws, S, stride, hL, ldws, ncols, gW, ldg, theta_w, g_theta, G, scale, ws2, S2, tail_tiles, ntail,
+                        plane, tail_first, w, ms, ms_theta, lr, rho, eps, clip, slice_, nslices, workgroups):
+        p = hip.ptr
+        hip.check(self.L.dcahip_heads_dw_update(p(ws), S, stride, hL, ldws, ncols, p(gW), ldg, p(theta_w), p(g_theta), G, scale,
+                                                p(ws2), S2, p(tail_tiles), ntail, plane, tail_first, p(w), p(ms), p(ms_theta),
+                                                p(lr), rho, eps, clip, slice_, nslices, workgroups, hip.stream()),
+                  'heads_dw_update')
+
     def counts_compact_ld(self, G):
         return int(self.L.dcahip_counts_compact_ld(G))
 
@@ -328,6 +340,17 @@
                                                       hip.ptr(ext_entries), hip.ptr(ext_counts), int(ext_E), hip.ptr(stat_out),
                                                       hip.ptr(ws), ws.numel() * ws.element_size(), hip.stream()),
                   'hidden_stack_fwd_sync')
+
+    def hidden_stack_bwd_ride(self, layers, B, n_total, act, dZ0, ldz0, step, ws, hL, G, plane, flags, gW, ldg, theta_w, g_theta,
+                              inv_n, ws_heads, tile_order, w, ms, ms_theta, lr, rho, eps, clip, nslices, rider_workgroups):
+        arr = self._bwd_layers(layers)
+        p = hip.ptr
+        hip.check(self.L.dcahip_hidden_stack_bwd_ride(arr, len(layers), B, float(n_total), int(act), p(dZ0), ldz0, int(step),
+                                                      p(ws), ws.numel() * ws.element_size(), hL, G, plane, flags, p(gW), ldg,
+                                                      p(theta_w), p(g_theta), inv_n, p(ws_heads),
+                                                      ws_heads.numel() * ws_heads.element_size(), p(tile_order), p(w), p(ms),
+                                                      p(ms_theta), p(lr), rho, eps, clip, int(step), int(nslices),
+                                                      int(rider_workgroups), hip.stream()), 'hidden_stack_bwd_ride')
 
     def hidden_stack_bwd_sync(self, layers, B, n_total, act, dZ0, ldz0, step, ext_sums, sums_out, ws):
         arr = self._bwd_layers(layers)
@@ -708,5 +731,12 @@
         hip.check(self.L.dcahip_rmsprop_clip(p(w), p(g), p(ms), n, p(lr), rho, eps, clip, p(loss), weight, p(hist),
                                              rows_per_slot, p(acc), p(cursor), advance, hip.stream()), 'rmsprop_clip')
 
+    def rmsprop_clip_skip_end(self, w, g, ms, n, skip0, skip1, lr, rho, eps, clip, loss, weight, hist, rows_per_slot, acc,
+                              cursor, advance):
+        p = hip.ptr
+        hip.check(self.L.dcahip_rmsprop_clip_skip(p(w), p(g), p(ms), n, skip0[0], skip0[1], skip1[0], skip1[1], p(lr), rho, eps,
+                                                  clip, p(loss), weight, p(hist), rows_per_slot, p(acc), p(cursor), advance,
+                                                  hip.stream()), 'rmsprop_clip_skip')
+
     def rmsprop_clip(self, w, g, ms, n, lr, rho, eps, clip):
         self.rmsprop_clip_end(w, g, ms, n, lr, rho, eps, clip, None, 0.0, None, 0, None, None, 0)
diff --git a/include/dcahip.h b/include/dcahip.h
--- a/include/dcahip.h
+++ b/include/dcahip.h
@@ -81,6 +81,23 @@
                        double* loss_partials, int* n_partials_out,
                        void* workspace, long workspace_bytes, const int* tile_order,
                        float* loss_out, int d_exp, void* stream);
+int dcahip_heads_fused_dw_partials(int B, int hL, int G, long plane, int flags);
+int dcahip_heads_fused_dh(const float* H, long ldh, const float* Wh, long ldw, const float* bh,
+                          long plane, const float* theta_w,
+                          const float* y, long ldy,
+                          const unsigned char* yc, long ldc, const int* ovf_ptr, const int* ovf_col,
+                          const float* ovf_val, const float* sf,
+                          const int* perm, const long long* cursor,
+                          int B, int hL, int G, float ridge, float inv_n, int flags,
+                          float* gW, long ldg, float* g_theta, float* dH, long lddh,
+                          double* loss_partials, int* n_partials_out,
+                          void* workspace, long workspace_bytes, const int* tile_order,
+                          float* loss_out, int d_exp, void* stream);
+int dcahip_heads_dw_update(const float* ws, int S, long stride, int hL, long ldws, long ncols, float* gW, long ldg,
+                           float* theta_w, float* g_theta, int G, float scale,
+                           const float* ws2, int S2, const int* tail_tiles, int ntail, long plane, int tail_first,
+                           float* w, float* ms, float* ms_theta, const float* lr, float rho, float eps, float clip,
+                           int slice, int nslices, int workgroups, void* stream);
 int dcahip_x3_product_32x32(const float* A, const float* B, float* C, int K, void* stream);
 
 int dcahip_sgemm(int ta, int tb, int M, int N, int K,
@@ -162,6 +179,13 @@
 int dcahip_hidden_stack_bwd(const dcahip_stack_bwd_layer* layers, int n, int B, float n_total, int act,
                             float* dZ0, long ldz0, int rows_per_wg, int first_step, int last_step,
                             void* workspace, long workspace_bytes, void* stream);
+int dcahip_hidden_stack_bwd_ride(const dcahip_stack_bwd_layer* layers, int n, int B, float n_total, int act,
+                                 float* dZ0, long ldz0, int step, void* workspace, long workspace_bytes,
+                                 int hL, int G, long plane, int flags, float* gW, long ldg,
+                                 float* theta_w, float* g_theta, float inv_n,
+                                 void* heads_workspace, long heads_workspace_bytes, const int* tile_order,
+                                 float* w, float* ms, float* ms_theta, const float* lr, float rho, float eps,
+                                 float clip, int slice, int nslices, int rider_workgroups, void* stream);
 
 int dcahip_hidden_stack_step_blocks(int B);
 int dcahip_hidden_stack_fwd_sync(const dcahip_small_layer* layers, int n, int B, float momentum, float eps, int act,
@@ -249,6 +273,11 @@
                         float rho, float eps, float clip, const float* loss, double weight,
                         float* hist, int rows_per_slot, double* acc, long long* cursor, int advance,
                         void* stream);
+int dcahip_rmsprop_clip_skip(float* w, const float* g, float* ms, long n, long skip0_lo, long skip0_hi,
+                             long skip1_lo, long skip1_hi, const float* lr,
+                             float rho, float eps, float clip, const float* loss, double weight,
+                             float* hist, int rows_per_slot, double* acc, long long* cursor, int advance,
+                             void* stream);
 
 #define DCAHIP_OPT_SGD       0
 #define DCAHIP_OPT_RMSPROP   1
```

Result: no change. 4.590 million, median of 6 (+0.4%).
